# jasonleebrown/machisplin

Hardware: AMD Instinct MI355X
Metric: grid Mcells/s (ensemble+TPS predict) + TPS-solve GFLOP/s (higher is better)
Workload: dtype f64; 1 GPU; cfg3: 5000 stations, 3 covariates, 10000x10000 grid, 6-model ensemble + TPS residual correction; stations=5000, covariates=3 x float32 planes resident in HBM, rf_trees=500, tps_mode=global (one fit on all stations, GCV lambda, V73:748-753), parallelism=rowband1 + bcast(coef) + 1 all-gather

## Files before the change

### machisplin_amd/csrc/ensemble.hip

```cpp
#include <algorithm>
#include <atomic>
#include <cmath>
#include <cstdio>
#include <cstdlib>
#include <cstring>
#include <functional>
#include <mutex>
#include <type_traits>
#include <vector>
#include "common.h"
#include "devmath.h"

#include "ensemble_int.h"

namespace mhs {

__global__ __launch_bounds__(256) void lm_kernel(const double *__restrict__ coef, int p, StackDev s,
                                                 PredGeom g, double weight, int accumulate,
                                                 double *__restrict__ out) {
    const int64_t i = (int64_t)blockIdx.x * 256 + threadIdx.x;
    if (i >= (int64_t)g.nr * g.nc) return;
    const int row = (int)(i / g.nc), col = (int)(i - (int64_t)row * g.nc);
    double acc = coef[0];
    for (int j = 0; j < p; ++j) acc = acc + coef[j + 1] * predictor(s, g, j, row, col);
    emit(out, (int64_t)row * g.ld_out + col, acc, weight, accumulate);
}

__device__ __forceinline__ double nnet_sigmoid(double z) {
    if (z < -15.0) return 0.0;
    if (z > 15.0) return 1.0;
    return 1.0 / (1.0 + exp(-z));
}

template <int P>
__global__ __launch_bounds__(256) void nnet_kernel(const double *__restrict__ w, int H, double y_scale,
                                                   double y_shift, StackDev s, PredGeom g,
                                                   double weight, int accumulate,
                                                   double *__restrict__ out) {
    const int64_t i = (int64_t)blockIdx.x * 256 + threadIdx.x;
    if (i >= (int64_t)g.nr * g.nc) return;
    const int row = (int)(i / g.nc), col = (int)(i - (int64_t)row * g.nc);
    double x[P];
    bool na = false;
#pragma unroll
    for (int j = 0; j < P; ++j) { x[j] = predictor(s, g, j, row, col); na |= isnan(x[j]); }
    double acc = w[(P + 1) * H];
    for (int h = 0; h < H; ++h) {
        const double *wh = w + h * (P + 1);
        double z = wh[0];
#pragma unroll
        for (int j = 0; j < P; ++j) z = z + wh[1 + j] * x[j];
        acc = acc + w[(P + 1) * H + 1 + h] * nnet_sigmoid(z);
    }
    acc = acc * y_scale + y_shift;
    emit(out, (int64_t)row * g.ld_out + col, na ? NAN : acc, weight, accumulate);
}

__global__ __launch_bounds__(256) void earth_kernel(const double *__restrict__ coef,
                                                    const double *__restrict__ fcut,
                                                    const int *__restrict__ tstart,
                                                    const int *__restrict__ fvar,
                                                    const int *__restrict__ fdir, int nterms, int p,
                                                    StackDev s, PredGeom g, double weight, int accumulate,
                                                    double *__restrict__ out) {
    const int64_t i = (int64_t)blockIdx.x * 256 + threadIdx.x;
    if (i >= (int64_t)g.nr * g.nc) return;
    const int row = (int)(i / g.nc), col = (int)(i - (int64_t)row * g.nc);
    bool na = false;
    for (int j = 0; j < p; ++j) na |= isnan(predictor(s, g, j, row, col));
    double acc = 0.0;
    for (int k = 0; k < nterms; ++k) {
        double term = 1.0;
        for (int f = tstart[k]; f < tstart[k + 1]; ++f) {
            const double xv = predictor(s, g, fvar[f], row, col);
            const int d = fdir[f];
            const double fac = d == 2 ? xv : (d == 1 ? fmax(0.0, xv - fcut[f]) : fmax(0.0, fcut[f] - xv));
            term = term * fac;
        }
        acc = acc + coef[k] * term;
    }
    emit(out, (int64_t)row * g.ld_out + col, na ? NAN : acc, weight, accumulate);
}

struct SmallArgs {
    const double *lm_coef;
    const double *nn_w; int nn_H; double nn_scale, nn_shift;
    const double *ea_coef; const double *ea_cut; const int *ea_tstart, *ea_fvar, *ea_fdir; int ea_nterms;
    double w_lm, w_nn, w_ea;
};
template <int P>
__global__ __launch_bounds__(256) void small_members_kernel(SmallArgs a, StackDev s, PredGeom g, int accumulate,
                                                            double *__restrict__ out) {
    const int64_t i = (int64_t)blockIdx.x * 256 + threadIdx.x;
    if (i >= (int64_t)g.nr * g.nc) return;
    const int row = (int)(i / g.nc), col = (int)(i - (int64_t)row * g.nc);
    double x[P];
    bool na = false;
#pragma unroll
    for (int j = 0; j < P; ++j) { x[j] = predictor(s, g, j, row, col); na |= isnan(x[j]); }
    const int64_t o = (int64_t)row * g.ld_out + col;
    double v = accumulate ? out[o] : 0.0;
    bool first = !accumulate;
    auto add = [&](double pred, double w) { const double t = pred * w; v = first ? t : v + t; first = false; };
    if (a.lm_coef) {
        double acc = a.lm_coef[0];
#pragma unroll
        for (int j = 0; j < P; ++j) acc = acc + a.lm_coef[j + 1] * x[j];
        add(acc, a.w_lm);
    }
    if (a.nn_w) {
        double acc = a.nn_w[(P + 1) * a.nn_H];
        for (int h = 0; h < a.nn_H; ++h) {
            const double *wh = a.nn_w + h * (P + 1);
            double z = wh[0];
#pragma unroll
            for (int j = 0; j < P; ++j) z = z + wh[1 + j] * x[j];
            acc = acc + a.nn_w[(P + 1) * a.nn_H + 1 + h] * nnet_sigmoid(z);
        }
        acc = acc * a.nn_scale + a.nn_shift;
        add(na ? NAN : acc, a.w_nn);
    }
    if (a.ea_coef) {
        double acc = 0.0;
        for (int k = 0; k < a.ea_nterms; ++k) {
            double term = 1.0;
            for (int f = a.ea_tstart[k]; f < a.ea_tstart[k + 1]; ++f) {
                const double xv = predictor(s, g, a.ea_fvar[f], row, col);
                const int d = a.ea_fdir[f];
                const double fac = d == 2 ? xv : (d == 1 ? fmax(0.0, xv - a.ea_cut[f]) : fmax(0.0, a.ea_cut[f] - xv));
                term = term * fac;
            }
            acc = acc + a.ea_coef[k] * term;
        }
        add(na ? NAN : acc, a.w_ea);
    }
    out[o] = v;
}

constexpr int EXP_TAB_BITS = 12;
constexpr int EXP_TAB_N = 1 << EXP_TAB_BITS;
constexpr double EXP_SCALE = 4096.0 / 0.6931471805599453094;
__device__ __forceinline__ double table_exp_neg_acc(double u, const double *tab, double acc) {
    const double MAGIC = 0x1.8p52 + 1023.0 * EXP_TAB_N, NK = -EXP_RANGE * EXP_SCALE;
    const double t = fma(u, NK, MAGIC);
    const double kd = t - MAGIC;
    unsigned k8 = (unsigned)__double2loint(t) << 8;
    asm("" : "+v"(k8));
    const double r = fma(u, NK, -kd);
    const double mj = *(const double *)((const char *)tab + __builtin_amdgcn_ubfe(k8, 5, EXP_TAB_BITS + 3));
    const double sj = __hiloint2double((int)((k8 & 0xfff00000u) | (unsigned)__double2hiint(mj)), __double2loint(mj));
    const double C1 = 1.0 / EXP_SCALE, C2 = 0.5 / (EXP_SCALE * EXP_SCALE);
    double q = fma(r, C2, C1);
    q = fma(q, r, 1.0);
    return fma(sj, q, acc);
}

#if defined(__HIP_DEVICE_COMPILE__) && !defined(__GFX9__)
#error "table_exp_neg_acc_rt relies on v_lshlrev_b16 zeroing bits 16..31 of its destination (GFX9 encoding only)"
#endif
constexpr int EXP_TAB2_N = 2 * EXP_TAB_N;
__device__ __forceinline__ void rt_exp_table_stage(double *tab2, const double *__restrict__ gtab, int tid, int nthreads) {
    for (int i = tid; i < EXP_TAB2_N; i += nthreads) {
        const int j = i & (EXP_TAB_N - 1);
        const double e = gtab[j];
        tab2[i] = __hiloint2double((int)(((unsigned)__double2hiint(e) & 0x000fffffu) - ((unsigned)j << 8)), __double2loint(e));
    }
}
constexpr double RT_EXP_MAGIC = 0x1.8p52 + 1023.0 * EXP_TAB_N, RT_EXP_C1 = 1.0 / EXP_SCALE;
__device__ __forceinline__ void rt_exp_consts(double &magic, double &c1) {
    magic = RT_EXP_MAGIC; c1 = RT_EXP_C1;
    asm("" : "+v"(magic));
    asm("" : "+v"(c1));
}
__device__ __forceinline__ double table_exp_neg_acc_rt(double u, const double *tab2, double acc, double magic, double c1) {
    const double MAGIC = RT_EXP_MAGIC, NK = -EXP_RANGE * EXP_SCALE;
    const double t = fma(u, NK, magic);
    const double kd = t - MAGIC;
    const unsigned k = (unsigned)__double2loint(t);
    unsigned off;
    asm("v_lshlrev_b16 %0, 3, %1" : "=v"(off) : "v"(k));
    const double r = fma(u, NK, -kd);
    const double mj = *(const double *)((const char *)tab2 + off);
    const double sj = __hiloint2double((int)((k << 8) + (unsigned)__double2hiint(mj)), __double2loint(mj));
    const double C2 = 0.5 / (EXP_SCALE * EXP_SCALE);
    double q = fma(r, C2, c1);
    q = fma(q, r, 1.0);
    return fma(sj, q, acc);
}

template <int P, int R>
__global__ __launch_bounds__(256) void svr_kernel(const double *__restrict__ svp, int nsv, int stride,
                                                  int npos, const double *__restrict__ xcs,
                                                  const double *__restrict__ gtab, double sigma, double b,
                                                  double amax,
                                                  double y_center, double y_scale, StackDev s, PredGeom g,
                                                  double weight, int accumulate, double *__restrict__ out) {
    __shared__ double etab[EXP_TAB_N];
    for (int i = threadIdx.x; i < EXP_TAB_N; i += 256) {
        const double e = gtab[i];
        etab[i] = __hiloint2double(__double2hiint(e) & 0x000fffff, __double2loint(e));
    }
    __syncthreads();
    const int64_t total = (int64_t)g.nr * g.nc;
    const int64_t half = (total + R - 1) / R;
    const int64_t i0 = (int64_t)blockIdx.x * 256 + threadIdx.x;
    if (i0 >= half) return;
    double x[R][P], q[R], acc[R];
    bool na[R];
    int row[R], col[R];
#pragma unroll
    for (int c = 0; c < R; ++c) {
        int64_t i = i0 + c * half;
        if (i >= total) i = total - 1;
        row[c] = (int)(i / g.nc); col[c] = (int)(i - (int64_t)row[c] * g.nc);
        na[c] = false; q[c] = 0.0; acc[c] = 0.0;
#pragma unroll
        for (int j = 0; j < P; ++j) {
            const double xv = predictor(s, g, j, row[c], col[c]);
            na[c] |= isnan(xv);
            x[c][j] = (xv - xcs[j]) / xcs[P + j];
            q[c] = fma(x[c][j], x[c][j], q[c]);
        }
        q[c] = (sigma / EXP_RANGE) * q[c];
    }
    double accn[R];
#pragma unroll
    for (int c = 0; c < R; ++c) accn[c] = 0.0;
    auto sum_range = [&](int v0, int v1, double (&a)[R]) {
        for (int v = v0; v < v1; ++v) {
            const double *sp = svp + (int64_t)v * stride;
#pragma unroll
            for (int c = 0; c < R; ++c) {
                double arg = q[c] + fma(sp[P - 1], x[c][P - 1], sp[P]);
#pragma unroll
                for (int j = 0; j < P - 1; ++j) arg = fma(sp[j], x[c][j], arg);
                arg = fmin(fmax(arg, 0.0), 1.0);
                a[c] = table_exp_neg_acc(arg, etab, a[c]);
            }
        }
    };
    sum_range(0, npos, acc);
    sum_range(npos, nsv, accn);
#pragma unroll
    for (int c = 0; c < R; ++c) {
        const int64_t i = i0 + c * half;
        if (i < total) {
            const double pred = ((acc[c] - accn[c]) * amax - b) * y_scale + y_center;
            emit(out, (int64_t)row[c] * g.ld_out + col[c], na[c] ? NAN : pred, weight, accumulate);
        }
    }
}

__device__ __attribute__((noinline)) double svr_rt_exp_call(double z) { return exp(z); }
template <int P, int R, bool TAB2, bool EXPCALL>
__device__ __forceinline__ void svr_rt_tile(const double *__restrict__ svp, int nsv, int stride, int npos,
                                            const double *__restrict__ xcs, const double *etab, double *aw, double sigma, double b,
                                            double amax, double y_center, double y_scale, const StackDev &s, const PredGeom &g,
                                            int row, int tcol, int lane, double weight, int accumulate, double *__restrict__ out) {
    constexpr int CH = 128;
    double x[R][P], q[R], acc[R], accn[R];
    bool na[R], ok[R];
    int col[R];
#pragma unroll
    for (int c = 0; c < R; ++c) {
        const int cc = tcol + c * 64 + lane;
        ok[c] = cc < g.nc;
        col[c] = min(cc, g.nc - 1);
        na[c] = false; q[c] = 0.0; acc[c] = 0.0; accn[c] = 0.0;
#pragma unroll
        for (int j = 0; j < P; ++j) {
            const double xv = predictor(s, g, j, row, col[c]);
            na[c] |= isnan(xv);
            x[c][j] = (xv - xcs[j]) / xcs[P + j];
            q[c] = fma(x[c][j], x[c][j], q[c]);
        }
        q[c] = (sigma / EXP_RANGE) * q[c];
    }
    const double xlat = x[0][P - 1];
    double qhi = -1.0, qlo = 2e300;
#pragma unroll
    for (int c = 0; c < R; ++c) { qhi = fmax(qhi, q[c]); qlo = fmin(qlo, q[c]); }
#pragma unroll
    for (int o = 32; o > 0; o >>= 1) { qhi = fmax(qhi, __shfl_xor(qhi, o)); qlo = fmin(qlo, __shfl_xor(qlo, o)); }
    const bool fold = __builtin_amdgcn_readfirstlane((int)(qhi - qlo <= 0.5)) != 0;
    const double S = fold ? qhi : 0.0;
    double magic = 0.0, c1 = 0.0;
    if constexpr (TAB2) rt_exp_consts(magic, c1);
    auto sum_range = [&](int v0, int v1, double (&a)[R], auto folded) {
        constexpr bool FOLD = decltype(folded)::value;
        auto pair = [&](const double *sp, const double ap) {
#pragma unroll
            for (int c = 0; c < R; ++c) {
                double arg = FOLD ? ap : q[c] + ap;
#pragma unroll
                for (int j = 0; j < P - 1; ++j) arg = fma(sp[j], x[c][j], arg);
                arg = fmin(fmax(arg, 0.0), 1.0);
                a[c] = TAB2 ? table_exp_neg_acc_rt(arg, etab, a[c], magic, c1) : table_exp_neg_acc(arg, etab, a[c]);
            }
        };
        for (int vb = v0; vb < v1; vb += CH) {
            const int n = min(CH, v1 - vb);
            __builtin_amdgcn_wave_barrier();
            for (int e = lane; e < n; e += 64) {
                const double *sp = svp + (int64_t)(vb + e) * stride;
                aw[e] = fma(sp[P - 1], xlat, sp[P]) + S;
            }
            __builtin_amdgcn_wave_barrier();
            const double *sp = svp + (int64_t)vb * stride;
            const double *ar = aw;
            int e = 0;
            for (; e + 4 <= n; e += 4) {
#pragma unroll
                for (int k = 0; k < 4; ++k) pair(sp + (int64_t)k * stride, ar[e + k]);
                sp += (int64_t)4 * stride;
            }
            for (; e < n; ++e) { pair(sp, ar[e]); sp += stride; }
        }
    };
    if (fold) {
        sum_range(0, npos, acc, std::true_type());
        sum_range(npos, nsv, accn, std::true_type());
    } else {
        sum_range(0, npos, acc, std::false_type());
        sum_range(npos, nsv, accn, std::false_type());
    }
#pragma unroll
    for (int c = 0; c < R; ++c)
        if (ok[c]) {
            const double back = fold ? (EXPCALL ? svr_rt_exp_call(EXP_RANGE * (S - q[c])) : exp(EXP_RANGE * (S - q[c]))) : 1.0;
            const double pred = ((acc[c] - accn[c]) * back * amax - b) * y_scale + y_center;
            emit(out, (int64_t)row * g.ld_out + col[c], na[c] ? NAN : pred, weight, accumulate);
        }
}

template <int P, int R, bool TAB2>
__device__ __forceinline__ void svr_rt_run(int64_t tile, const double *__restrict__ svp, int nsv, int stride, int npos,
                                           const double *__restrict__ xcs, const double *etab, double *aw, double sigma, double b,
                                           double amax, double y_center, double y_scale, const StackDev &s, const PredGeom &g,
                                           int tiles_per_row, int lane, double weight, int accumulate, double *__restrict__ out) {
    const int row = (int)(tile / tiles_per_row), tcol = (int)(tile - (int64_t)row * tiles_per_row) * (64 * R);
    svr_rt_tile<P, R, TAB2, true>(svp, nsv, stride, npos, xcs, etab, aw, sigma, b, amax, y_center, y_scale, s, g, row, tcol, lane, weight,
                                  accumulate, out);
}
template <int NW, bool TAB2>
__device__ __forceinline__ void svr_rt_stage(double *etab, const double *__restrict__ gtab) {
    if constexpr (TAB2) rt_exp_table_stage(etab, gtab, threadIdx.x, 64 * NW);
    else
        for (int i = threadIdx.x; i < EXP_TAB_N; i += 64 * NW) {
            const double e = gtab[i];
            etab[i] = __hiloint2double(__double2hiint(e) & 0x000fffff, __double2loint(e));
        }
}

template <int P, int R, int NW, bool TAB2>
__global__ __launch_bounds__(64 * NW) void svr_rt_kernel(const double *__restrict__ svp, int nsv, int stride,
                                                         int npos, const double *__restrict__ xcs,
                                                         const double *__restrict__ gtab, double sigma, double b,
                                                         double amax, double y_center, double y_scale, StackDev s, PredGeom g,
                                                         int tiles_per_row, double weight, int accumulate, double *__restrict__ out) {
    __shared__ double etab[TAB2 ? EXP_TAB2_N : EXP_TAB_N];
    __shared__ double aw[NW][128];
    svr_rt_stage<NW, TAB2>(etab, gtab);
    __syncthreads();
    const int wave = threadIdx.x >> 6, lane = threadIdx.x & 63;
    const int64_t ntiles = (int64_t)g.nr * tiles_per_row;
    const int64_t tile = (int64_t)blockIdx.x * NW + wave;
    if (tile >= ntiles) return;
    const int row = (int)(tile / tiles_per_row), tcol = (int)(tile - (int64_t)row * tiles_per_row) * (64 * R);
    svr_rt_tile<P, R, TAB2, false>(svp, nsv, stride, npos, xcs, etab, aw[wave], sigma, b, amax, y_center, y_scale, s, g, row, tcol, lane,
                                   weight, accumulate, out);
}

struct SvrRtScalars {
    int nsv, stride, npos, tiles_per_row; double sigma, b, amax, y_center, y_scale;
    StackDev s; PredGeom g; double weight; int accumulate;
};
constexpr int SVR_RT_SCALARS_AT = 5 * sizeof(void *);
static_assert(alignof(SvrRtScalars) <= 8, "svr_rt_resident_kernel: `sc` does not follow the pointers without padding");
static_assert(sizeof(PredGeom) == 64 && sizeof(StackDev) == 48 && sizeof(SvrRtScalars) == 184,
              "svr_rt_resident_kernel copies PredGeom / StackDev field by field: update the copies and these sizes together");
inline void svr_rt_field_counts(const PredGeom &g, const StackDev &s) {
    const auto &[g0, g1, g2, g3, g4, g5, g6, g7, g8] = g;
    const auto &[s0, s1, s2, s3, s4, s5, s6, s7] = s;
    (void)g0; (void)g1; (void)g2; (void)g3; (void)g4; (void)g5; (void)g6; (void)g7; (void)g8;
    (void)s0; (void)s1; (void)s2; (void)s3; (void)s4; (void)s5; (void)s6; (void)s7;
}
template <int P, int R, int NW, bool TAB2, int WPS>
__global__ __launch_bounds__(64 * NW, WPS) void svr_rt_resident_kernel(const double *__restrict__ svp, const double *__restrict__ xcs,
                                                                  const double *__restrict__ gtab, double *__restrict__ out,
                                                                  unsigned long long *__restrict__ pool, SvrRtScalars sc) {
    __shared__ double etab[TAB2 ? EXP_TAB2_N : EXP_TAB_N];
    __shared__ double aw[NW][128];
    svr_rt_stage<NW, TAB2>(etab, gtab);
    __syncthreads();
    const int wave = threadIdx.x >> 6, lane = threadIdx.x & 63;
    typedef const __attribute__((address_space(4))) char *KBytes;
    typedef const __attribute__((address_space(4))) SvrRtScalars *KScalars;
    for (;;) {
        KScalars k = (KScalars)((KBytes)__builtin_amdgcn_kernarg_segment_ptr() + SVR_RT_SCALARS_AT);
        asm volatile("" : "+s"(k));
        unsigned long long t = 0;
        if (lane == 0) t = atomicAdd(pool, 1ull);
        const int64_t tile = (int64_t)(((unsigned long long)(unsigned)__builtin_amdgcn_readfirstlane((int)(t >> 32)) << 32) |
                                       (unsigned)__builtin_amdgcn_readfirstlane((int)t));
        const PredGeom g = {k->g.xmin, k->g.ymax, k->g.xres, k->g.yres, k->g.r0, k->g.c0, k->g.nr, k->g.nc, k->g.ld_out};
        if (tile >= (int64_t)g.nr * k->tiles_per_row) return;
        const StackDev s = {k->s.data, k->s.C, k->s.dtype, k->s.plane_stride, k->s.ld, k->s.nodata, k->s.has_nodata, k->s.all_from_planes};
        svr_rt_run<P, R, TAB2>(tile, svp, k->nsv, k->stride, k->npos, xcs, etab, aw[wave], k->sigma, k->b, k->amax,
                               k->y_center, k->y_scale, s, g, k->tiles_per_row, lane, k->weight, k->accumulate, out);
    }
}

template <bool GBM, bool LDS_NODES, int R, bool NA_ONLY, bool SPLIT = false>
__global__ __launch_bounds__(256) void tree_kernel(const Node *__restrict__ gnodes,
                                                   const int *__restrict__ tree_off,
                                                   const TreeChunk *__restrict__ chunks, int n_chunks,
                                                   int n_trees, double init_f, int p, StackDev s,
                                                   PredGeom g, double weight, int accumulate,
                                                   double *__restrict__ out, const unsigned *__restrict__ na_gate = nullptr) {
    extern __shared__ __attribute__((aligned(16))) char smem[];
    if (NA_ONLY && na_gate && na_gate[1] == 0u) return;
    double *xs = (double *)smem;
    Node *lnodes = (Node *)(smem + (size_t)p * R * 256 * sizeof(double));
    const int64_t total = (int64_t)g.nr * g.nc;
    const int64_t half = (total + R - 1) / R;
    const int64_t i0 = (int64_t)blockIdx.x * 256 + threadIdx.x;
    int row[R], col[R];
    bool na[R];
    double acc[R];
#pragma unroll
    for (int c = 0; c < R; ++c) {
        int64_t i = i0 + c * half;
        if (i >= total) i = total - 1;
        if (i < 0) i = 0;
        row[c] = (int)(i / g.nc); col[c] = (int)(i - (int64_t)row[c] * g.nc);
        na[c] = false; acc[c] = 0.0;
        for (int j = 0; j < p; ++j) {
            const double xv = predictor(s, g, j, row[c], col[c]);
            na[c] |= isnan(xv);
            xs[(j * R + c) * 256 + threadIdx.x] = xv;
        }
    }
    if (NA_ONLY) {
        bool any = false;
#pragma unroll
        for (int c = 0; c < R; ++c) any |= na[c] && i0 < half && (i0 + c * half) < total;
        if (!__syncthreads_or(any)) return;
    }
    int ch_begin = 0, ch_end = n_chunks;
    if (SPLIT) {
        const int per = (n_chunks + (int)gridDim.y - 1) / (int)gridDim.y;
        ch_begin = min((int)blockIdx.y * per, n_chunks);
        ch_end = min(ch_begin + per, n_chunks);
    }
    for (int ch = ch_begin; ch < ch_end; ++ch) {
        const TreeChunk tc = chunks[ch];
        if (LDS_NODES) {
            __syncthreads();
            const int4 *src = (const int4 *)(gnodes + tc.node_begin);
            int4 *dst = (int4 *)lnodes;
            for (int e = threadIdx.x; e < tc.node_count; e += 256) dst[e] = src[e];
            __syncthreads();
        }
        for (int t = tc.first_tree; t < tc.first_tree + tc.n_trees; ++t) {
            const int tbase = LDS_NODES ? tree_off[t] - tc.node_begin : tree_off[t];
#pragma unroll
            for (int c = 0; c < R; ++c) {
                if (NA_ONLY && !na[c]) continue;
                Node nd;
                if constexpr (LDS_NODES) nd = lnodes[tbase]; else nd = gnodes[tbase];
                while (nd.var >= 0) {
                    const double xv = xs[(nd.var * R + c) * 256 + threadIdx.x];
                    unsigned nxt;
                    if (GBM) nxt = isnan(xv) ? nd.missing : (xv < nd.val ? nd.left : nd.right);
                    else nxt = (xv <= nd.val) ? nd.left : nd.right;
                    if constexpr (LDS_NODES) nd = lnodes[tbase + nxt]; else nd = gnodes[tbase + nxt];
                }
                acc[c] = acc[c] + nd.val;
            }
        }
    }
    if (SPLIT) {
#pragma unroll
        for (int c = 0; c < R; ++c) {
            const int64_t i = i0 + c * half;
            if (i0 < half && i < total) out[(int64_t)blockIdx.y * total + i] = (!GBM && na[c]) ? NAN : acc[c];
        }
        return;
    }
#pragma unroll
    for (int c = 0; c < R; ++c) {
        const int64_t i = i0 + c * half;
        if (i0 < half && i < total && (!NA_ONLY || na[c])) {
            double pred;
            if (GBM) pred = init_f + acc[c];
            else pred = na[c] ? NAN : acc[c] / (double)n_trees;
            emit(out, (int64_t)row[c] * g.ld_out + col[c], pred, weight, accumulate);
        }
    }
}


__global__ __launch_bounds__(256) void na_collect_kernel(StackDev s, PredGeom g, unsigned cap, unsigned *__restrict__ list) {
    const int64_t total = (int64_t)g.nr * g.nc;
    const int64_t i = (int64_t)blockIdx.x * 256 + threadIdx.x;
    if (i >= total) return;
    const int row = (int)(i / g.nc), col = (int)(i - (int64_t)row * g.nc);
    bool na = false;
    for (int j = 0; j < s.C; ++j) na |= isnan(predictor(s, g, j, row, col));
    if (na) {
        const unsigned slot = atomicAdd(&list[0], 1u);
        if (slot < cap) list[2 + slot] = (unsigned)i;
        else list[1] = 1u;
    }
}
template <bool LDS_NODES>
__global__ __launch_bounds__(256) void gbm_na_list_kernel(const Node *__restrict__ gnodes, const int *__restrict__ tree_off,
                                                          const TreeChunk *__restrict__ chunks, int n_chunks, double init_f, int p,
                                                          StackDev s, PredGeom g, double weight, int accumulate,
                                                          double *__restrict__ out, const unsigned *__restrict__ list, unsigned cap) {
    extern __shared__ __attribute__((aligned(16))) char smem[];
    if (list[1]) return;
    double *xs = (double *)smem;
    Node *lnodes = (Node *)(smem + (size_t)p * 256 * sizeof(double));
    const unsigned count = min(list[0], cap);
    for (unsigned base = blockIdx.x * 256u; base < count; base += gridDim.x * 256u) {
        const bool live = base + threadIdx.x < count;
        const int64_t i = list[2 + (live ? base + threadIdx.x : base)];
        const int row = (int)(i / g.nc), col = (int)(i - (int64_t)row * g.nc);
        for (int j = 0; j < p; ++j) xs[j * 256 + threadIdx.x] = predictor(s, g, j, row, col);
        double acc = 0.0;
        for (int ch = 0; ch < n_chunks; ++ch) {
            const TreeChunk tc = chunks[ch];
            if (LDS_NODES) {
                __syncthreads();
                const int4 *src = (const int4 *)(gnodes + tc.node_begin);
                int4 *dst = (int4 *)lnodes;
                for (int e = threadIdx.x; e < tc.node_count; e += 256) dst[e] = src[e];
                __syncthreads();
            }
            for (int t = tc.first_tree; t < tc.first_tree + tc.n_trees; ++t) {
                const int tbase = LDS_NODES ? tree_off[t] - tc.node_begin : tree_off[t];
                Node nd;
                if constexpr (LDS_NODES) nd = lnodes[tbase]; else nd = gnodes[tbase];
                while (nd.var >= 0) {
                    const double xv = xs[nd.var * 256 + threadIdx.x];
                    const unsigned nxt = isnan(xv) ? nd.missing : (xv < nd.val ? nd.left : nd.right);
                    if constexpr (LDS_NODES) nd = lnodes[tbase + nxt]; else nd = gnodes[tbase + nxt];
                }
                acc = acc + nd.val;
            }
        }
        if (live) emit(out, (int64_t)row * g.ld_out + col, init_f + acc, weight, accumulate);
        __syncthreads();
    }
}


template <bool HI>
__device__ __forceinline__ void pred_bits(float2v &b01, float2v &b23, const float2v k01, const float2v k23,
                                          const unsigned long long cpair) {
    if (!HI)
        asm("v_pk_add_f32 %0, %2, %4 op_sel_hi:[1,0] clamp\n\t"
            "v_pk_add_f32 %1, %3, %4 op_sel_hi:[1,0] clamp"
            : "=&v"(b01), "=&v"(b23) : "v"(k01), "v"(k23), "s"(cpair));
    else
        asm("v_pk_add_f32 %0, %2, %4 op_sel:[0,1] op_sel_hi:[1,1] clamp\n\t"
            "v_pk_add_f32 %1, %3, %4 op_sel:[0,1] op_sel_hi:[1,1] clamp"
            : "=&v"(b01), "=&v"(b23) : "v"(k01), "v"(k23), "s"(cpair));
}


template <int S>
__global__ __launch_bounds__(256) void gbm_lut_kernel(const double *__restrict__ lut,
                                                      const int *__restrict__ meta,
                                                      const void *__restrict__ sorted, int key64,
                                                      const int *__restrict__ sorted_off, int n_trees_padded,
                                                      double init_f, int p, StackDev s, PredGeom g,
                                                      double weight, int accumulate,
                                                      double *__restrict__ out) {
    static_assert((LUT_CHUNK << S) * sizeof(double) >= LUT_COARSE * sizeof(float), "coarse table must fit");
    extern __shared__ __attribute__((aligned(16))) char smem[];
    float *keys = (float *)smem;
    double *slut = (double *)(smem + (size_t)p * 256 * LUT_R * sizeof(float));
    float *coarse = (float *)slut;
    const int64_t total = (int64_t)g.nr * g.nc;
    const int64_t quarter = (total + LUT_R - 1) / LUT_R;
    const int64_t i0 = (int64_t)blockIdx.x * 256 + threadIdx.x;
    int row[LUT_R], col[LUT_R];
    bool na[LUT_R];
    double acc[LUT_R];
#pragma unroll
    for (int c = 0; c < LUT_R; ++c) {
        int64_t i = i0 + c * quarter;
        if (i >= total) i = total - 1;
        row[c] = (int)(i / g.nc); col[c] = (int)(i - (int64_t)row[c] * g.nc);
        na[c] = false; acc[c] = 0.0;
    }
    for (int j = 0; j < p; ++j) {
        float r[LUT_R];
        lut_ranks<LUT_R, 256>(j, sorted, key64, sorted_off, coarse, s, g, row, col, na, r);
#pragma unroll
        for (int c = 0; c < LUT_R; ++c) keys[(j * 256 + threadIdx.x) * LUT_R + c] = -r[c];
    }
    const char *kbase = (const char *)(keys + threadIdx.x * LUT_R);
    constexpr unsigned A0_BITS = (unsigned)(127 + 23 - S) << 23;
    unsigned lut_base = (unsigned)p * 256u * LUT_R * (unsigned)sizeof(float) - 0x58000000u;
    asm volatile("" : "+s"(lut_base));
    for (int t0 = 0; t0 < n_trees_padded; t0 += LUT_CHUNK) {
        __syncthreads();
        for (int e = threadIdx.x; e < (LUT_CHUNK << S); e += 256) slut[e] = lut[((int64_t)t0 << S) + e];
        __syncthreads();
#pragma unroll 2
        for (int t = 0; t < LUT_CHUNK; ++t) {
            const int *m = meta + (int64_t)(t0 + t) * LUT_META_DW;
            const unsigned long long *mc = (const unsigned long long *)m;
            const unsigned long long a0 = A0_BITS + ((unsigned)t << S);
            float2v a01, a23, b01, b23;
            {
                const float4 k = *(const float4 *)(kbase + m[6]);
                pred_bits<false>(b01, b23, float2v{k.x, k.y}, float2v{k.z, k.w}, mc[0]);
                asm("v_pk_fma_f32 %0, %2, 2.0, %3 op_sel_hi:[0,0,1]\n\t"
                    "v_pk_fma_f32 %1, %2, 2.0, %4 op_sel_hi:[0,0,1]"
                    : "=&v"(a01), "=&v"(a23) : "s"(a0), "v"(b01), "v"(b23));
            }
#pragma unroll
            for (int q = 1; q < S; ++q) {
                const float4 k = *(const float4 *)(kbase + m[6 + q]);
                if (q & 1) pred_bits<true>(b01, b23, float2v{k.x, k.y}, float2v{k.z, k.w}, mc[q >> 1]);
                else pred_bits<false>(b01, b23, float2v{k.x, k.y}, float2v{k.z, k.w}, mc[q >> 1]);
                asm("v_pk_fma_f32 %0, %0, 2.0, %2 op_sel_hi:[1,0,1]\n\t"
                    "v_pk_fma_f32 %1, %1, 2.0, %3 op_sel_hi:[1,0,1]"
                    : "+v"(a01), "+v"(a23) : "v"(b01), "v"(b23));
            }
            acc[0] = acc[0] + *(const double *)(smem + (__float_as_uint(a01.x) * 8u + lut_base));
            acc[1] = acc[1] + *(const double *)(smem + (__float_as_uint(a01.y) * 8u + lut_base));
            acc[2] = acc[2] + *(const double *)(smem + (__float_as_uint(a23.x) * 8u + lut_base));
            acc[3] = acc[3] + *(const double *)(smem + (__float_as_uint(a23.y) * 8u + lut_base));
        }
    }
#pragma unroll
    for (int c = 0; c < LUT_R; ++c) {
        const int64_t i = i0 + c * quarter;
        if (i0 < quarter && i < total && !na[c])
            emit(out, (int64_t)row[c] * g.ld_out + col[c], init_f + acc[c], weight, accumulate);
    }
}

typedef float float32v __attribute__((ext_vector_type(32)));
constexpr int LUT_REG_P = 8;

#define MHS_LUT_LEVEL(IDX, CP, SEL)                                                   \
    "s_set_gpr_idx_idx %[" IDX "]\n\t"                                               \
    "v_pk_add_f32 %[b01], v[64:65], %[" CP "] " SEL " clamp\n\t"                     \
    "v_pk_add_f32 %[b23], v[66:67], %[" CP "] " SEL " clamp\n\t"                     \
    "v_pk_fma_f32 %[a01], 2.0, %[a01], %[b01] op_sel_hi:[0,1,1]\n\t"                 \
    "v_pk_fma_f32 %[a23], 2.0, %[a23], %[b23] op_sel_hi:[0,1,1]\n\t"
#define MHS_SEL_LO "op_sel_hi:[1,0]"
#define MHS_SEL_HI "op_sel:[0,1] op_sel_hi:[1,1]"

template <int S>
__device__ __forceinline__ void lut_tree_reg(float2v &a01, float2v &a23, const float32v &keys, const int *m,
                                             const unsigned long long a0) {
    const unsigned long long *mc = (const unsigned long long *)m;
    const unsigned long long c01 = mc[0], c23 = mc[1], c45 = mc[2];
    const int i0 = m[6] >> 10, i1 = m[7] >> 10, i2 = m[8] >> 10, i3 = m[9] >> 10, i4 = m[10] >> 10;
    float2v b01, b23;
    if (S == 5) {
        asm("s_set_gpr_idx_on %[i0], 0x1\n\t"
            "v_pk_add_f32 %[b01], v[64:65], %[c01] op_sel_hi:[1,0] clamp\n\t"
            "v_pk_add_f32 %[b23], v[66:67], %[c01] op_sel_hi:[1,0] clamp\n\t"
            "v_pk_fma_f32 %[a01], 2.0, %[a0], %[b01] op_sel_hi:[0,0,1]\n\t"
            "v_pk_fma_f32 %[a23], 2.0, %[a0], %[b23] op_sel_hi:[0,0,1]\n\t"
            MHS_LUT_LEVEL("i1", "c01", MHS_SEL_HI)
            MHS_LUT_LEVEL("i2", "c23", MHS_SEL_LO)
            MHS_LUT_LEVEL("i3", "c23", MHS_SEL_HI)
            MHS_LUT_LEVEL("i4", "c45", MHS_SEL_LO)
            "s_set_gpr_idx_off"
            : [a01] "=&v"(a01), [a23] "=&v"(a23), [b01] "=&v"(b01), [b23] "=&v"(b23)
            : "{v[64:95]}"(keys), [i0] "s"(i0), [i1] "s"(i1), [i2] "s"(i2), [i3] "s"(i3), [i4] "s"(i4),
              [c01] "s"(c01), [c23] "s"(c23), [c45] "s"(c45), [a0] "s"(a0));
    } else {
        const int i5 = m[11] >> 10;
        asm("s_set_gpr_idx_on %[i0], 0x1\n\t"
            "v_pk_add_f32 %[b01], v[64:65], %[c01] op_sel_hi:[1,0] clamp\n\t"
            "v_pk_add_f32 %[b23], v[66:67], %[c01] op_sel_hi:[1,0] clamp\n\t"
            "v_pk_fma_f32 %[a01], 2.0, %[a0], %[b01] op_sel_hi:[0,0,1]\n\t"
            "v_pk_fma_f32 %[a23], 2.0, %[a0], %[b23] op_sel_hi:[0,0,1]\n\t"
            MHS_LUT_LEVEL("i1", "c01", MHS_SEL_HI)
            MHS_LUT_LEVEL("i2", "c23", MHS_SEL_LO)
            MHS_LUT_LEVEL("i3", "c23", MHS_SEL_HI)
            MHS_LUT_LEVEL("i4", "c45", MHS_SEL_LO)
            MHS_LUT_LEVEL("i5", "c45", MHS_SEL_HI)
            "s_set_gpr_idx_off"
            : [a01] "=&v"(a01), [a23] "=&v"(a23), [b01] "=&v"(b01), [b23] "=&v"(b23)
            : "{v[64:95]}"(keys), [i0] "s"(i0), [i1] "s"(i1), [i2] "s"(i2), [i3] "s"(i3), [i4] "s"(i4), [i5] "s"(i5),
              [c01] "s"(c01), [c23] "s"(c23), [c45] "s"(c45), [a0] "s"(a0));
    }
}

template <int S, bool K64>
__global__ __launch_bounds__(256, 5) void gbm_lutreg_kernel(const double *__restrict__ lut,
                                                         const int *__restrict__ meta,
                                                         const void *__restrict__ sorted, int key64,
                                                         const int *__restrict__ sorted_off, int n_trees_padded,
                                                         double init_f, int p, StackDev s, PredGeom g,
                                                         double weight, int accumulate,
                                                         double *__restrict__ out) {
    static_assert((LUT_CHUNK << S) * sizeof(double) >= LUT_COARSE * sizeof(float), "coarse table must fit");
    extern __shared__ __attribute__((aligned(16))) char smem[];
    double *slut = (double *)smem;
    float *coarse = (float *)smem;
    const int64_t total = (int64_t)g.nr * g.nc;
    const int64_t quarter = (total + LUT_R - 1) / LUT_R;
    const int64_t i0 = (int64_t)blockIdx.x * 256 + threadIdx.x;
    int row[LUT_R], col[LUT_R];
    bool na[LUT_R];
    double acc[LUT_R];
#pragma unroll
    for (int c = 0; c < LUT_R; ++c) {
        int64_t i = i0 + c * quarter;
        if (i >= total) i = total - 1;
        row[c] = (int)(i / g.nc); col[c] = (int)(i - (int64_t)row[c] * g.nc);
        na[c] = false; acc[c] = 0.0;
    }
    float32v keys;
#pragma unroll
    for (int j = 0; j < LUT_REG_P; ++j) {
        float r[LUT_R] = {0.f, 0.f, 0.f, 0.f};
        if (j < p) {
            if constexpr (K64) lut_ranks_t<LUT_R, 256, double>(j, (const double *)sorted, sorted_off, (double *)coarse, s, g, row, col, na, r);
            else lut_ranks_t<LUT_R, 256, float>(j, (const float *)sorted, sorted_off, coarse, s, g, row, col, na, r);
        }
#pragma unroll
        for (int c = 0; c < LUT_R; ++c) keys[j * LUT_R + c] = -r[c];
    }
    constexpr unsigned A0_BITS = (unsigned)(127 + 23 - S) << 23;
    unsigned lut_base = 0u - 0x58000000u;
    asm volatile("" : "+s"(lut_base));
    for (int t0 = 0; t0 < n_trees_padded; t0 += LUT_CHUNK) {
        __syncthreads();
        for (int e = threadIdx.x; e < (LUT_CHUNK << S); e += 256) slut[e] = lut[((int64_t)t0 << S) + e];
        __syncthreads();
#pragma unroll 2
        for (int t = 0; t < LUT_CHUNK; ++t) {
            float2v a01, a23;
            lut_tree_reg<S>(a01, a23, keys, meta + (int64_t)(t0 + t) * LUT_META_DW, A0_BITS + ((unsigned)t << S));
            acc[0] = acc[0] + *(const double *)(smem + (__float_as_uint(a01.x) * 8u + lut_base));
            acc[1] = acc[1] + *(const double *)(smem + (__float_as_uint(a01.y) * 8u + lut_base));
            acc[2] = acc[2] + *(const double *)(smem + (__float_as_uint(a23.x) * 8u + lut_base));
            acc[3] = acc[3] + *(const double *)(smem + (__float_as_uint(a23.y) * 8u + lut_base));
        }
    }
#pragma unroll
    for (int c = 0; c < LUT_R; ++c) {
        const int64_t i = i0 + c * quarter;
        if (i0 < quarter && i < total && !na[c])
            emit(out, (int64_t)row[c] * g.ld_out + col[c], init_f + acc[c], weight, accumulate);
    }
}

constexpr int LUT_RT_DW = 16;
constexpr int LUT_RT_MAXK = 2;
typedef unsigned long long u64x8 __attribute__((ext_vector_type(8)));

constexpr int GBC_PROBE_BLOCKS = 4, GBC_PROBE_CHUNKS = 4, GBC_PROBE_SLOTS = 1024;
__device__ __forceinline__ bool gbc_coherent_pays(const int *__restrict__ probe) {
    long long cost = 0, cnt = 0;
#pragma unroll
    for (int b = 0; b < GBC_PROBE_BLOCKS; ++b) { cost += probe[2 * b]; cnt += probe[2 * b + 1]; }
    return cost < 83 * cnt;
}
template <bool K64>
__global__ __launch_bounds__(256, 5) void gbm_lutreg_rt_kernel(const double *__restrict__ lut,
                                                            const u64x8 *__restrict__ meta,
                                                            const void *__restrict__ sorted,
                                                            const int *__restrict__ sorted_off, int n_trees_padded,
                                                            double init_f, int p, StackDev s, PredGeom g, int tiles_per_row,
                                                            double weight, int accumulate,
                                                            double *__restrict__ out, const int *__restrict__ probe) {
    constexpr int S = 5;
    static_assert((LUT_CHUNK << S) * sizeof(double) >= LUT_COARSE * sizeof(float), "coarse table must fit");
    extern __shared__ __attribute__((aligned(16))) char smem[];
    if (probe && gbc_coherent_pays(probe)) return;
    double *slut = (double *)smem;
    float *coarse = (float *)smem;
    const int lane = threadIdx.x & 63;
    const int64_t ntiles = (int64_t)g.nr * tiles_per_row;
    int64_t tile = (int64_t)blockIdx.x * 4 + (threadIdx.x >> 6);
    const bool live = tile < ntiles;
    if (!live) tile = ntiles - 1;
    const int trow = (int)(tile / tiles_per_row), tcol = (int)(tile - (int64_t)trow * tiles_per_row) * (64 * LUT_R);
    int row[LUT_R], col[LUT_R];
    bool na[LUT_R], ok[LUT_R];
    double acc[LUT_R];
#pragma unroll
    for (int c = 0; c < LUT_R; ++c) {
        const int cc = tcol + c * 64 + lane;
        ok[c] = live && cc < g.nc;
        row[c] = trow; col[c] = min(cc, g.nc - 1);
        na[c] = false; acc[c] = 0.0;
    }
    float32v keys;
    int latv = 0;
#pragma unroll
    for (int j = 0; j < LUT_REG_P; ++j) {
        float r[LUT_R] = {0.f, 0.f, 0.f, 0.f};
        if (j < p) {
            if constexpr (K64) lut_ranks_t<LUT_R, 256, double>(j, (const double *)sorted, sorted_off, (double *)coarse, s, g, row, col, na, r);
            else lut_ranks_t<LUT_R, 256, float>(j, (const float *)sorted, sorted_off, coarse, s, g, row, col, na, r);
            if (j == s.C + 1) latv = (int)r[0];
        }
#pragma unroll
        for (int c = 0; c < LUT_R; ++c) keys[j * LUT_R + c] = -r[c];
    }
    const int latrank = __builtin_amdgcn_readfirstlane(latv);
    unsigned lut_base = 0u - 0x58000000u;
    asm volatile("" : "+s"(lut_base));
    for (int t0 = 0; t0 < n_trees_padded; t0 += LUT_CHUNK) {
        __syncthreads();
        for (int e = threadIdx.x; e < (LUT_CHUNK << S); e += 256) slut[e] = lut[((int64_t)t0 << S) + e];
        __syncthreads();
        const u64x8 *mp = meta + t0;
        asm volatile(
#include "gbm_rt_loop.inc"
            : [acc0] "+v"(acc[0]), [acc1] "+v"(acc[1]), [acc2] "+v"(acc[2]), [acc3] "+v"(acc[3])
            : "{v[64:95]}"(keys), [mp] "s"(mp), [lat] "s"(latrank), [lb] "s"(lut_base)
            : "memory", "scc",
              "s36", "s37", "s38", "s39", "s40", "s41", "s42", "s43", "s44", "s45", "s46", "s47", "s48", "s49", "s50", "s51",
              "s52", "s53", "s54", "s55", "s56", "s57", "s58", "s59", "s60", "s61", "s62", "s63", "s64", "s65", "s66", "s67",
              "s68", "s69", "s70", "s71", "s72", "s73", "s74",
              "v40", "v41", "v42", "v43", "v44", "v45", "v46", "v47", "v48", "v49", "v50", "v51", "v52", "v53", "v54", "v55",
              "v56", "v57", "v58", "v59");
    }
#pragma unroll
    for (int c = 0; c < LUT_R; ++c)
        if (ok[c] && !na[c]) emit(out, (int64_t)row[c] * g.ld_out + col[c], init_f + acc[c], weight, accumulate);
}


constexpr int GBC_WAVES = 16;
__device__ __forceinline__ double gbc_lds_f64(unsigned a) { return *(__attribute__((address_space(3))) const double *)(uintptr_t)a; }
typedef float float4v __attribute__((ext_vector_type(4)));
template <bool K64, bool PROBE = false>
__global__ __launch_bounds__(1024) void gbm_coherent_kernel(const double *__restrict__ lut, const unsigned *__restrict__ cls,
                                                            const void *__restrict__ sorted, const int *__restrict__ sorted_off,
                                                            int n_trees_padded, double init_f, int p, StackDev s, PredGeom g,
                                                            int tiles_per_row, double weight, int accumulate,
                                                            double *__restrict__ out, int *__restrict__ probe, int tile16,
                                                            const int *__restrict__ axis_rank, int axis_ncol) {
    constexpr int S = 5, CH = LUT_CHUNK, CLS_STRIDE = 384, R = LUT_R;
    if (!PROBE && probe && !gbc_coherent_pays(probe)) return;
    if (PROBE) n_trees_padded = min(n_trees_padded, GBC_PROBE_CHUNKS * CH);
    static_assert(R == 4, "four cells per lane: two packed predicate instructions");
    static_assert((CH << S) * sizeof(double) >= LUT_COARSE * sizeof(float), "coarse table must fit");
    extern __shared__ __attribute__((aligned(16))) char smem[];
    double *slut = (double *)smem;
    unsigned *scls = (unsigned *)(smem + 2 * (CH << S) * sizeof(double));
    int2 *srange = (int2 *)(scls + 2 * CLS_STRIDE);
    float *coarse = (float *)smem;
    if ((unsigned)(uintptr_t)(__attribute__((address_space(3))) char *)smem != 0u) __builtin_trap();
    const int tid = threadIdx.x, wave = tid >> 6, lane = tid & 63;
    const int TW = tile16 ? 16 : 64, TH = tile16 ? 4 * R : R;
    const int roff = (int)(g.r0 % TH), coff = (int)(g.c0 % TW);
    const int64_t ntiles = (int64_t)((g.nr + roff + TH - 1) / TH) * tiles_per_row;
    int64_t tile = (int64_t)blockIdx.x * GBC_WAVES + wave;
    if (PROBE) tile = ntiles >= GBC_PROBE_BLOCKS * GBC_WAVES ? tile * (ntiles / (GBC_PROBE_BLOCKS * GBC_WAVES)) : tile % ntiles;
    const bool live = tile < ntiles;
    if (!live) tile = ntiles - 1;
    const int trow = (int)(tile / tiles_per_row) * TH - roff + (tile16 ? (lane >> 4) * R : 0);
    const int tcol = (int)(tile % tiles_per_row) * TW - coff + (tile16 ? (lane & 15) : lane);
    int row[R], col[R];
    bool na[R], ok[R];
    double acc[R];
#pragma unroll
    for (int c = 0; c < R; ++c) {
        const int rr = trow + c, cc = tcol;
        ok[c] = live && cc >= 0 && cc < g.nc && rr >= 0 && rr < g.nr;
        row[c] = min(max(rr, 0), g.nr - 1); col[c] = min(max(cc, 0), g.nc - 1);
        na[c] = false; acc[c] = 0.0;
    }
    float32v keys;
#pragma unroll
    for (int j = 0; j < LUT_REG_P; ++j) {
        float r[R] = {0.f, 0.f, 0.f, 0.f};
        if (j < p) {
            if (axis_rank && j >= s.C && !s.all_from_planes) {
#pragma unroll
                for (int c = 0; c < R; ++c)
                    r[c] = (float)(j == s.C ? axis_rank[g.c0 + col[c]] : axis_rank[(int64_t)axis_ncol + g.r0 + row[c]]);
            } else if constexpr (K64) lut_ranks_t<R, 1024, double>(j, (const double *)sorted, sorted_off, (double *)coarse, s, g, row, col, na, r);
            else lut_ranks_t<R, 1024, float>(j, (const float *)sorted, sorted_off, coarse, s, g, row, col, na, r);
        }
#pragma unroll
        for (int c = 0; c < R; ++c) keys[j * R + c] = -r[c];
        int mn = 0x7fffffff, mx = -1;
#pragma unroll
        for (int c = 0; c < R; ++c)
            if (!na[c]) { mn = min(mn, (int)r[c]); mx = max(mx, (int)r[c]); }
#pragma unroll
        for (int o = 32; o > 0; o >>= 1) { mn = min(mn, __shfl_xor(mn, o)); mx = max(mx, __shfl_xor(mx, o)); }
        if (lane == 0) srange[wave * 8 + j] = make_int2(mn, mx);
    }
    __syncthreads();
    for (int e = tid; e < (CH << S); e += 1024) slut[e] = lut[e];
    if (tid < CH * S) scls[tid] = cls[tid];
    __syncthreads();
    double usum = 0.0;
    int pcost = 0;
    for (int t0 = 0, buf = 0; t0 < n_trees_padded; t0 += CH, buf ^= 1) {
        const bool more = t0 + CH < n_trees_padded;
        double pre0 = 0.0, pre1 = 0.0;
        unsigned prec = 0u;
        if (more) {
            const double *ln = lut + ((int64_t)(t0 + CH) << S);
            pre0 = ln[tid]; pre1 = ln[tid + 1024];
            if (tid < CH * S) prec = cls[(int64_t)(t0 + CH) * S + tid];
        }
        const unsigned *cw = scls + buf * CLS_STRIDE + lane * S;
        const double *L = slut + buf * (CH << S) + (lane << S);
        unsigned w[S];
        int2 mm[S];
#pragma unroll
        for (int q = 0; q < S; ++q) w[q] = cw[q];
#pragma unroll
        for (int q = 0; q < S; ++q) mm[q] = srange[wave * 8 + (int)(w[q] & 7u)];
        unsigned known = 0u, smask = 0u;
#pragma unroll
        for (int q = 0; q < S; ++q) {
            const int c = (int)(w[q] >> 3);
            const bool all1 = mm[q].y < c, all0 = mm[q].x >= c;
            if (all1) known |= 16u >> q;
            if (!(all1 || all0)) smask |= 16u >> q;
        }
        const unsigned nstr = (unsigned)__popc(smask);
        if (PROBE) {
            if (nstr) pcost += 85 + 26 * (int)nstr;
            if (more) {
                double *ld = slut + (buf ^ 1) * (CH << S);
                ld[tid] = pre0; ld[tid + 1024] = pre1;
                if (tid < CH * S) scls[(buf ^ 1) * CLS_STRIDE + tid] = prec;
            }
            __syncthreads();
            continue;
        }
        const double B = L[known];
        const bool single = nstr == 1u, pair = nstr == 2u, multi = nstr >= 3u;
        if (!multi) usum = usum + B;
        double d1 = 0.0, d2 = 0.0, d12 = 0.0;
        unsigned f1 = 0u, f2 = 0u;
        if (single || pair) {
            const int pos1 = 31 - __clz((int)(smask | 1u));
            const unsigned p1 = 1u << pos1;
            f1 = cw[S - 1 - pos1];
            const double A1 = L[known + p1];
            d1 = (A1 - B) * 128.0;
            if (pair) {
                const int pos2 = 31 - __clz((int)((smask & ~p1) | 1u));
                const unsigned p2 = 1u << pos2;
                f2 = cw[S - 1 - pos2];
                const double A2 = L[known + p2], A12 = L[known + p1 + p2];
                d2 = (A2 - B) * 128.0;
                d12 = (((A12 - A1) - A2) + B) * 16384.0;
            }
            f1 = __float_as_uint((float)(int)(f1 >> 3)) | (f1 & 7u);
            f2 = __float_as_uint((float)(int)(f2 >> 3)) | (f2 & 7u);
        }
#define MHS_GBC_RL(x) __builtin_amdgcn_readlane((int)(x), t)
#define MHS_GBC_RLD(x) __hiloint2double(__builtin_amdgcn_readlane(__double2hiint(x), t), __builtin_amdgcn_readlane(__double2loint(x), t))
#define MHS_GBC_THR(fw) (int)((unsigned)(fw) & ~7u)
#define MHS_GBC_VO(fw) (int)(((unsigned)(fw) & 7u) << 2)
#define MHS_GBC_BITS(h0, h1, h2, h3, vo, cc)                                                                 \
        asm volatile("s_set_gpr_idx_on %[v], 0x1\n\t"                                                        \
                     "v_add_f32_e64 %[a], v64, %[c] clamp\n\t"                                               \
                     "v_add_f32_e64 %[b], v65, %[c] clamp\n\t"                                               \
                     "v_add_f32_e64 %[d], v66, %[c] clamp\n\t"                                               \
                     "v_add_f32_e64 %[e], v67, %[c] clamp\n\t"                                               \
                     "s_set_gpr_idx_off"                                                                     \
                     : [a] "=&v"(h0), [b] "=&v"(h1), [d] "=&v"(h2), [e] "=&v"(h3)                            \
                     : "{v[64:95]}"(keys), [v] "s"(vo), [c] "s"(cc));
        for (unsigned long long m1 = __builtin_amdgcn_ballot_w64(single); m1; m1 &= m1 - 1ull) {
            const int t = (int)__builtin_ctzll(m1);
            const int fw = MHS_GBC_RL(f1);
            const int cc = MHS_GBC_THR(fw), vo = MHS_GBC_VO(fw);
            const double e1 = MHS_GBC_RLD(d1);
            int h[R];
            MHS_GBC_BITS(h[0], h[1], h[2], h[3], vo, cc)
#pragma unroll
            for (int c = 0; c < R; ++c) acc[c] = fma(__hiloint2double(h[c], 0), e1, acc[c]);
        }
        for (unsigned long long mp = __builtin_amdgcn_ballot_w64(pair); mp; mp &= mp - 1ull) {
            const int t = (int)__builtin_ctzll(mp);
            const int fa = MHS_GBC_RL(f1), fb = MHS_GBC_RL(f2);
            const int c1 = MHS_GBC_THR(fa), v1 = MHS_GBC_VO(fa), c2 = MHS_GBC_THR(fb), v2 = MHS_GBC_VO(fb);
            const double e1 = MHS_GBC_RLD(d1), e2 = MHS_GBC_RLD(d2), e12 = MHS_GBC_RLD(d12);
            int h[R], k[R];
            MHS_GBC_BITS(h[0], h[1], h[2], h[3], v1, c1)
            MHS_GBC_BITS(k[0], k[1], k[2], k[3], v2, c2)
#pragma unroll
            for (int c = 0; c < R; ++c) {
                const double b1 = __hiloint2double(h[c], 0), b2 = __hiloint2double(k[c], 0);
                acc[c] = fma(b1, e1, acc[c]);
                acc[c] = fma(b2, fma(b1, e12, e2), acc[c]);
            }
        }
#undef MHS_GBC_BITS
#undef MHS_GBC_RLD
        const unsigned abase = (unsigned)buf * (unsigned)((CH << S) * sizeof(double)) - 0x58000000u;
        unsigned long long m2 = __builtin_amdgcn_ballot_w64(multi);
        unsigned wf[S];
#pragma unroll
        for (int q = 0; q < S; ++q) wf[q] = w[q];
        if (m2) {
#pragma unroll
            for (int q = 0; q < S; ++q) wf[q] = __float_as_uint((float)(int)(w[q] >> 3)) | (w[q] & 7u);
        }
        for (; m2; m2 &= m2 - 1ull) {
            const int t = (int)__builtin_ctzll(m2);
            const unsigned sm = (unsigned)MHS_GBC_RL(smask);
            const float a0 = __uint_as_float(0x4B000000u + ((unsigned)t << S) + (unsigned)MHS_GBC_RL(known));
            float2v s01 = {a0, a0}, s23 = {a0, a0};
#pragma unroll
            for (int q = 0; q < S; ++q) {
                if (sm & (16u >> q)) {
                    const int fw = MHS_GBC_RL(wf[q]);
                    const unsigned long long cc = (unsigned)MHS_GBC_THR(fw);
                    const int vo = MHS_GBC_VO(fw);
                    const unsigned long long wb = (127u + (unsigned)(S - 1 - q)) << 23;
                    float2v b01, b23;
                    asm volatile("s_set_gpr_idx_on %[vo], 0x1\n\t"
                                 "v_pk_add_f32 %[b01], v[64:65], %[cc] op_sel_hi:[1,0] clamp\n\t"
                                 "v_pk_add_f32 %[b23], v[66:67], %[cc] op_sel_hi:[1,0] clamp\n\t"
                                 "s_set_gpr_idx_off\n\t"
                                 "v_pk_fma_f32 %[s01], %[b01], %[wb], %[s01] op_sel_hi:[1,0,1]\n\t"
                                 "v_pk_fma_f32 %[s23], %[b23], %[wb], %[s23] op_sel_hi:[1,0,1]"
                                 : [s01] "+v"(s01), [s23] "+v"(s23), [b01] "=&v"(b01), [b23] "=&v"(b23)
                                 : "{v[64:95]}"(keys), [vo] "s"(vo), [cc] "s"(cc), [wb] "s"(wb));
                }
            }
            acc[0] = acc[0] + gbc_lds_f64(__float_as_uint(s01.x) * 8u + abase);
            acc[1] = acc[1] + gbc_lds_f64(__float_as_uint(s01.y) * 8u + abase);
            acc[2] = acc[2] + gbc_lds_f64(__float_as_uint(s23.x) * 8u + abase);
            acc[3] = acc[3] + gbc_lds_f64(__float_as_uint(s23.y) * 8u + abase);
        }
#undef MHS_GBC_VO
#undef MHS_GBC_THR
#undef MHS_GBC_RL
        if (more) {
            double *ld = slut + (buf ^ 1) * (CH << S);
            ld[tid] = pre0; ld[tid + 1024] = pre1;
            if (tid < CH * S) scls[(buf ^ 1) * CLS_STRIDE + tid] = prec;
        }
        __syncthreads();
    }
    if (PROBE) {
        int *tot = (int *)srange;
        __syncthreads();
        if (tid == 0) tot[0] = 0;
        __syncthreads();
#pragma unroll
        for (int o = 32; o > 0; o >>= 1) pcost += __shfl_xor(pcost, o);
        if (lane == 0) atomicAdd(tot, pcost);
        __syncthreads();
        if (tid == 0) { probe[2 * blockIdx.x] = tot[0]; probe[2 * blockIdx.x + 1] = GBC_WAVES * n_trees_padded; }
        return;
    }
#pragma unroll
    for (int o = 32; o > 0; o >>= 1) usum = usum + __shfl_xor(usum, o);
#pragma unroll
    for (int c = 0; c < R; ++c)
        if (ok[c] && !na[c]) emit(out, (int64_t)row[c] * g.ld_out + col[c], init_f + (acc[c] + usum), weight, accumulate);
}
static size_t gbc_lds_bytes() {
    return 2 * ((size_t)LUT_CHUNK << 5) * sizeof(double) + 2 * 384 * sizeof(unsigned) + GBC_WAVES * 8 * sizeof(int2);
}

__global__ __launch_bounds__(256) void gbm_staged_points_kernel(const Node *__restrict__ nodes, const int *__restrict__ tree_off,
                                                                int n_trees, double init_f, const double *__restrict__ X,
                                                                int64_t n, int step, double *__restrict__ out) {
    const int64_t i = (int64_t)blockIdx.x * 256 + threadIdx.x;
    if (i >= n) return;
    double acc = 0.0;
    for (int t = 0; t < n_trees; ++t) {
        const int tb = tree_off[t];
        Node nd = nodes[tb];
        while (nd.var >= 0) {
            const double xv = X[(int64_t)nd.var * n + i];
            const unsigned nxt = isnan(xv) ? nd.missing : (xv < nd.val ? nd.left : nd.right);
            nd = nodes[tb + nxt];
        }
        acc = acc + nd.val;
        if ((t + 1) % step == 0) out[(int64_t)((t + 1) / step - 1) * n + i] = init_f + acc;
    }
}

struct ResidualArgs { double w[8]; };
__global__ __launch_bounds__(256) void residual_points_kernel(const double *__restrict__ pred, const double *__restrict__ resp,
                                                              int64_t n, int n_models, ResidualArgs a, double wt_total,
                                                              double *__restrict__ out) {
    const int64_t i = (int64_t)blockIdx.x * 256 + threadIdx.x;
    if (i >= n) return;
    const double y = resp[i];
    double res = (y - pred[i]) * a.w[0];
    for (int k = 1; k < n_models; ++k) res = res + (y - pred[(int64_t)k * n + i]) * a.w[k];
    out[i] = res / wt_total;
}

__global__ __launch_bounds__(256) void scale_add_kernel(const double *__restrict__ a, double divisor,
                                                        const double *__restrict__ b,
                                                        double *__restrict__ out, int64_t n) {
    const int64_t i = (int64_t)blockIdx.x * 256 + threadIdx.x;
    if (i >= n) return;
    double v = a[i] / divisor;
    if (b) v = v + b[i];
    out[i] = v;
}

__global__ __launch_bounds__(256) void scale_window_kernel(double *__restrict__ out, int nr, int nc,
                                                           int64_t ld, double divisor) {
    const int64_t i = (int64_t)blockIdx.x * 256 + threadIdx.x;
    if (i >= (int64_t)nr * nc) return;
    const int row = (int)(i / nc), col = (int)(i - (int64_t)row * nc);
    out[(int64_t)row * ld + col] = out[(int64_t)row * ld + col] / divisor;
}


template <int P>
static void launch_nnet(const mhs_model *m, const StackDev &s, const PredGeom &g, double w, int acc,
                        double *out, hipStream_t st, unsigned blocks) {
    hipLaunchKernelGGL((nnet_kernel<P>), dim3(blocks), dim3(256), 0, st, m->dpar, m->n0, m->s0, m->s1, s, g, w, acc, out);
}
constexpr bool svr_rt_tab2(int P) { return P <= 5; }
constexpr int svr_rt_waves_per_simd(int P) { return P <= 5 ? 4 : 3; }
constexpr int svr_rt_waves(int P) { return svr_rt_tab2(P) ? 16 : 4; }

static std::mutex svr_pool_mu[MAX_SLOTS];
static int svr_pool_take(Context &c, hipStream_t st, int *idx, unsigned long long **counter) {
    if (!c.svr_pool) {
        for (hipEvent_t &e : c.svr_pool_ev)
            if (!e) MHS_HIP(hipEventCreateWithFlags(&e, hipEventDisableTiming));
        MHS_HIP(hipMalloc((void **)&c.svr_pool, sizeof(unsigned long long) * SVR_POOL_SLOTS));
    }
    *idx = (int)(c.svr_pool_next++ % SVR_POOL_SLOTS);
    *counter = c.svr_pool + *idx;
    MHS_HIP(hipStreamWaitEvent(st, c.svr_pool_ev[*idx], 0));
    MHS_HIP(hipMemsetAsync(*counter, 0, sizeof(unsigned long long), st));
    return MHS_OK;
}

template <int P>
static int launch_svr(const mhs_model *m, const StackDev &s, const PredGeom &g, double w, int acc,
                      double *out, hipStream_t st, int64_t total) {
    constexpr int R = 3;
    const int tpr = (g.nc + 64 * R - 1) / (64 * R);
    if (!s.all_from_planes && P == s.C + 2 && P >= 3 && !getenv("MHS_SVR_NO_ROWTILE") && (double)g.nc >= 0.93 * (double)tpr * (64 * R)) {
        const int64_t ntiles = (int64_t)g.nr * tpr;
        constexpr int NW = svr_rt_waves(P);
        const int64_t covering = (ntiles + NW - 1) / NW;
        if constexpr (svr_rt_tab2(P)) {
            auto kern = svr_rt_resident_kernel<P, R, NW, true, svr_rt_waves_per_simd(P)>;
            Context &c = ctx();
            std::lock_guard<std::mutex> lk(svr_pool_mu[current_slot()]);
            int &per_cu = c.svr_rt_blocks_per_cu[P];
            if (per_cu == 0) {
                int n = 0;
                MHS_HIP(hipOccupancyMaxActiveBlocksPerMultiprocessor(&n, (const void *)kern, 64 * NW, 0));
                per_cu = std::max(1, n);
            }
            const int64_t resident = (int64_t)(c.n_cu > 0 ? c.n_cu : 256) * per_cu;
            int idx = 0;
            unsigned long long *counter = nullptr;
            if (int rc = svr_pool_take(c, st, &idx, &counter)) return rc;
            const SvrRtScalars sc = {m->n0, m->n1, m->n2, tpr, m->s1, m->s0, m->s4, m->s2, m->s3, s, g, w, acc};
            hipLaunchKernelGGL(kern, dim3((unsigned)std::min(resident, covering)), dim3(64 * NW), 0, st,
                               m->dpar, m->dpar + (size_t)m->n0 * m->n1, c.exp_tab, out, counter, sc);
            MHS_HIP(hipEventRecord(c.svr_pool_ev[idx], st));
            return MHS_OK;
        }
        else {
            hipLaunchKernelGGL((svr_rt_kernel<P, R, NW, false>), dim3((unsigned)covering), dim3(64 * NW), 0, st,
                               m->dpar, m->n0, m->n1, m->n2, m->dpar + (size_t)m->n0 * m->n1, ctx().exp_tab, m->s1, m->s0, m->s4,
                               m->s2, m->s3, s, g, tpr, w, acc, out);
            return MHS_OK;
        }
    }
    const int64_t half = (total + R - 1) / R;
    hipLaunchKernelGGL((svr_kernel<P, R>), dim3((unsigned)((half + 255) / 256)), dim3(256), 0, st,
                       m->dpar, m->n0, m->n1, m->n2, m->dpar + (size_t)m->n0 * m->n1, ctx().exp_tab, m->s1, m->s0, m->s4,
                       m->s2, m->s3,
                       s, g, w, acc, out);
    return MHS_OK;
}

#define MHS_DISPATCH_P(P_, CALL)                                                     \
    switch (P_) {                                                                    \
        case 2: CALL(2); break; case 3: CALL(3); break; case 4: CALL(4); break;      \
        case 5: CALL(5); break; case 6: CALL(6); break; case 7: CALL(7); break;      \
        case 8: CALL(8); break; case 9: CALL(9); break; case 10: CALL(10); break;    \
        case 11: CALL(11); break; case 12: CALL(12); break;                          \
        default: set_error("predict: p = %d exceeds the %d predictors this build supports for nnet/ksvm", P_, PMAX); \
                 return MHS_ERR_INVALID;                                             \
    }

template <bool GBM>
__global__ __launch_bounds__(256) void tree_finalize_kernel(const double *__restrict__ part, int shares, int64_t total,
                                                            double init_f, int n_trees, PredGeom g, double weight,
                                                            int accumulate, double *__restrict__ out) {
    const int64_t i = (int64_t)blockIdx.x * 256 + threadIdx.x;
    if (i >= total) return;
    double acc = 0.0;
    for (int y = 0; y < shares; ++y) acc = acc + part[(int64_t)y * total + i];
    const int row = (int)(i / g.nc), col = (int)(i - (int64_t)row * g.nc);
    emit(out, (int64_t)row * g.ld_out + col, GBM ? init_f + acc : acc / (double)n_trees, weight, accumulate);
}

constexpr int64_t TREE_SPLIT_MAX_CELLS = 16384;
constexpr int TREE_SPLIT_SHARES = 64;

template <typename K, typename... Args>
static int launch_tree_kernel(const mhs_model *m, K lds_kern, K global_kern, dim3 blocks, size_t xs_bytes, hipStream_t st, Args... args) {
    const K kern = m->lds_ok ? lds_kern : global_kern;
    const size_t bytes = xs_bytes + (m->lds_ok ? (size_t)m->max_chunk_nodes * sizeof(Node) : 0);
    MHS_HIP(hipFuncSetAttribute((const void *)kern, hipFuncAttributeMaxDynamicSharedMemorySize, (int)bytes));
    hipLaunchKernelGGL(kern, blocks, dim3(256), bytes, st, args...);
    return MHS_OK;
}

template <bool GBM, bool NA_ONLY>
static int launch_trees(const mhs_model *m, const StackDev &s, const PredGeom &g, double w, int acc,
                        double *out, hipStream_t st, int64_t total, const unsigned *na_gate = nullptr) {
    const size_t xs_bytes = (size_t)m->p * TREE_R * 256 * sizeof(double);
    if (xs_bytes > LDS_MAX) {
        const size_t xs1 = (size_t)m->p * 256 * sizeof(double);
        const auto kern = tree_kernel<GBM, false, 1, NA_ONLY>;
        MHS_HIP(hipFuncSetAttribute((const void *)kern, hipFuncAttributeMaxDynamicSharedMemorySize, (int)xs1));
        hipLaunchKernelGGL(kern, dim3((unsigned)((total + 255) / 256)), dim3(256), xs1, st, m->nodes, m->tree_off, m->chunks, m->n_chunks,
                           m->n_trees, m->init_f, m->p, s, g, w, acc, out, na_gate);
        return MHS_OK;
    }
    const int64_t half = (total + TREE_R - 1) / TREE_R;
    const unsigned blocks = (unsigned)((half + 255) / 256);
    if (!NA_ONLY && m->lds_ok && total <= TREE_SPLIT_MAX_CELLS && m->n_chunks >= 4) {
        const int shares = std::min(m->n_chunks, TREE_SPLIT_SHARES);
        mhs_model *mm = const_cast<mhs_model *>(m);
        if (!mm->split_scratch) MHS_HIP(hipMalloc((void **)&mm->split_scratch, sizeof(double) * TREE_SPLIT_MAX_CELLS * TREE_SPLIT_SHARES));
        auto kern = tree_kernel<GBM, true, TREE_R, false, true>;
        if (int rc = launch_tree_kernel(m, kern, kern, dim3(blocks, (unsigned)shares), xs_bytes, st, m->nodes, m->tree_off, m->chunks,
                                        m->n_chunks, m->n_trees, m->init_f, m->p, s, g, w, acc, mm->split_scratch, (const unsigned *)nullptr))
            return rc;
        hipLaunchKernelGGL(tree_finalize_kernel<GBM>, dim3((unsigned)((total + 255) / 256)), dim3(256), 0, st,
                           mm->split_scratch, shares, total, m->init_f, m->n_trees, g, w, acc, out);
        return MHS_OK;
    }
    return launch_tree_kernel(m, tree_kernel<GBM, true, TREE_R, NA_ONLY>, tree_kernel<GBM, false, TREE_R, NA_ONLY>, dim3(blocks), xs_bytes, st,
                              m->nodes, m->tree_off, m->chunks, m->n_chunks, m->n_trees, m->init_f, m->p, s, g, w, acc, out, na_gate);
}

template <typename KT>
static int build_lut_meta_t(mhs_model *m, const mhs_grid &grid, int C) {
    const int S = m->lut_S;
    std::vector<KT> tkey((size_t)m->n_trees * S, (KT)0);
    std::vector<std::vector<KT>> sorted((size_t)m->p);
    for (int t = 0; t < m->n_trees; ++t) {
        for (int q = 0; q < S; ++q) {
            const int v = m->lut_var[(size_t)t * S + q];
            if (v < 0) continue;
            const KT tk = split_tkey<KT, false>(v, C, m->lut_thr[(size_t)t * S + q], grid);
            tkey[(size_t)t * S + q] = tk;
            sorted[(size_t)v].push_back(tk);
        }
    }
    std::vector<int> off;
    std::vector<KT> flat;
    sort_unique(sorted, off, flat);
    for (int v = 0; v < m->p; ++v)
        if (sorted[(size_t)v].size() >= ((size_t)1 << 24)) { set_error("gbm: too many distinct split values"); return MHS_ERR_INVALID; }
    if (int rc = publish_axis_ranks(m, sorted, C, grid)) return rc;
    std::vector<int> meta((size_t)m->n_trees_padded * LUT_META_DW, 0);
    const float never = -33554432.f;
    for (int t = 0; t < m->n_trees_padded; ++t) {
        int *mt = &meta[(size_t)t * LUT_META_DW];
        for (int q = 0; q < 6; ++q) { memcpy(&mt[q], &never, 4); mt[6 + q] = 0; }
        if (t >= m->n_trees) continue;
        for (int q = 0; q < S; ++q) {
            const int v = m->lut_var[(size_t)t * S + q];
            if (v < 0) continue;
            const std::vector<KT> &sv = sorted[(size_t)v];
            const KT tk = tkey[(size_t)t * S + q];
            const float c = (float)((std::lower_bound(sv.begin(), sv.end(), tk) - sv.begin()) + 1);
            memcpy(&mt[q], &c, 4);
            mt[6 + q] = v * 256 * LUT_R * (int)sizeof(float);
        }
    }
    if (m->p <= LUT_REG_P && S == 5 && !m->lut_host.empty()) {
        const int lat = C + 1 < m->p ? C + 1 : -2;
        std::vector<int> rmeta(((size_t)m->n_trees_padded + 1) * LUT_RT_DW, 0);
        std::vector<double> rlut(m->lut_host.size(), 0.0);
        for (int t = 0; t <= m->n_trees_padded; ++t) {
            int *mt = &rmeta[(size_t)t * LUT_RT_DW];
            for (int q = 0; q < 5; ++q) { memcpy(&mt[q], &never, 4); mt[6 + q] = 0; mt[11 + q] = 0; }
            mt[5] = S - LUT_RT_MAXK;
            if (t >= m->n_trees) continue;
            int perm[6], K = 0, n = 0;
            bool first[6] = {false, false, false, false, false, false};
            for (int q = 0; q < S && K < LUT_RT_MAXK; ++q) {
                const int v = m->lut_var[(size_t)t * S + q];
                if (v < 0 || v == lat) { perm[n++] = q; first[q] = true; ++K; }
            }
            for (int q = 0; q < S; ++q) if (!first[q]) perm[n++] = q;
            for (int i = 0; i < S; ++i) {
                const int q = perm[i], v = m->lut_var[(size_t)t * S + q];
                if (v < 0) continue;
                const std::vector<KT> &sv = sorted[(size_t)v];
                const int c = (int)(std::lower_bound(sv.begin(), sv.end(), tkey[(size_t)t * S + q]) - sv.begin()) + 1;
                if (i < K) mt[11 + i] = c;
                else { const float cf = (float)c; memcpy(&mt[i - K], &cf, 4); mt[6 + i - K] = v * LUT_R; }
            }
            mt[5] = S - K;
            for (int b = 0; b < (1 << S); ++b) {
                int bo = 0;
                for (int i = 0; i < S; ++i) bo |= ((b >> (S - 1 - i)) & 1) << (S - 1 - perm[i]);
                rlut[((size_t)t << S) + b] = m->lut_host[((size_t)t << S) + bo];
            }
        }
        if (int rc = publish(m, rlut, &m->lut_rt)) return rc;
        if (int rc = publish(m, rmeta, &m->lut_rt_meta)) return rc;
        std::vector<unsigned> cw((size_t)m->n_trees_padded * 5, 0u);
        for (int t = 0; t < m->n_trees; ++t)
            for (int q = 0; q < S; ++q) {
                const int v = m->lut_var[(size_t)t * S + q];
                if (v < 0) continue;
                const std::vector<KT> &sv = sorted[(size_t)v];
                const unsigned c = (unsigned)(std::lower_bound(sv.begin(), sv.end(), tkey[(size_t)t * S + q]) - sv.begin()) + 1u;
                cw[(size_t)t * 5 + q] = (c << 3) | (unsigned)v;
            }
        bool fits = true;
        for (int v = 0; v < m->p; ++v) fits = fits && sorted[(size_t)v].size() < ((size_t)1 << 20);
        if (fits) { if (int rc = publish(m, cw, &m->lut_cls)) return rc; }
        else if (m->lut_cls) { m->retired.push_back((void *)m->lut_cls); m->lut_cls = nullptr; }
    }
    if (int rc = publish(m, flat, (KT **)&m->lut_sorted)) return rc;
    if (int rc = publish(m, off, &m->lut_sorted_off)) return rc;
    return publish(m, meta, &m->lut_meta);
}

static int build_lut_meta(mhs_model *m, const mhs_grid &grid, int C, int key64, TreeTables *tt) {
    std::lock_guard<std::mutex> lk(m->mu);
    if (!(m->lut_meta && same_meta(m, grid, C, key64))) {
        if (int rc = key64 ? build_lut_meta_t<double>(m, grid, C) : build_lut_meta_t<float>(m, grid, C)) return rc;
        m->meta_grid = grid; m->meta_C = C; m->meta_key64 = key64;
    }
    *tt = TreeTables{m->lut_sorted, m->lut_sorted_off, m->lut_meta, nullptr, nullptr, m->lut_rt, m->lut_rt_meta, m->lut_cls, m->axis_rank, m->axis_ncol};
    return MHS_OK;
}

static int launch_gbm_na(const mhs_model *m, const StackDev &s, const PredGeom &g, double w, int acc, double *out, hipStream_t st,
                         int64_t total) {
    if (total >= (1LL << 32)) return launch_trees<true, true>(m, s, g, w, acc, out, st, total);
    mhs_model *mm = const_cast<mhs_model *>(m);
    const unsigned slot = mm->na_next.fetch_add(1) % 4;
    const size_t want = (size_t)std::max<int64_t>(4096, total / 8);
    unsigned *list = nullptr;
    unsigned cap = 0;
    {
        std::lock_guard<std::mutex> lk(mm->mu);
        if (!mm->na_done[slot]) MHS_HIP(hipEventCreateWithFlags(&mm->na_done[slot], hipEventDisableTiming));
        else if (mm->na_stream[slot] != st) MHS_HIP(hipStreamWaitEvent(st, mm->na_done[slot], 0));
        if (mm->na_cap[slot] < want) {
            if (mm->na_list[slot]) {
                MHS_HIP(hipEventSynchronize(mm->na_done[slot]));
                MHS_HIP(hipStreamSynchronize(st));
                (void)hipFree(mm->na_list[slot]); mm->na_list[slot] = nullptr; mm->na_cap[slot] = 0;
            }
            MHS_HIP(hipMalloc((void **)&mm->na_list[slot], sizeof(unsigned) * (want + 2)));
            mm->na_cap[slot] = want;
        }
        list = mm->na_list[slot];
        cap = (unsigned)mm->na_cap[slot];
        mm->na_stream[slot] = st;
    }
    MHS_HIP(hipMemsetAsync(list, 0, 2 * sizeof(unsigned), st));
    hipLaunchKernelGGL(na_collect_kernel, dim3((unsigned)((total + 255) / 256)), dim3(256), 0, st, s, g, cap, list);
    const unsigned lblocks = (unsigned)std::min<int64_t>(2048, (total / 8 + 255) / 256 + 1);
    if (int rc = launch_tree_kernel(m, gbm_na_list_kernel<true>, gbm_na_list_kernel<false>, dim3(lblocks), (size_t)m->p * 256 * sizeof(double), st,
                                    m->nodes, m->tree_off, m->chunks, m->n_chunks, m->init_f, m->p, s, g, w, acc, out, list, cap))
        return rc;
    if (int rc = launch_trees<true, true>(m, s, g, w, acc, out, st, total, list)) return rc;
    MHS_HIP(hipGetLastError());
    {
        std::lock_guard<std::mutex> lk(mm->mu);
        MHS_HIP(hipEventRecord(mm->na_done[slot], st));
    }
    return MHS_OK;
}

static bool gbm_lut_applies(const mhs_model *m, const StackDev &s, const mhs_grid *grid) {
    return grid && m->lut_S > 0 && !s.all_from_planes && !getenv("MHS_TREES_GENERIC") &&
           (size_t)m->p * 256 * LUT_R * 4 + ((size_t)LUT_CHUNK << m->lut_S) * 8 <= LDS_LIMIT;
}

static int launch_gbm_lut(const mhs_model *m, const StackDev &s, const PredGeom &g, const mhs_grid &grid,
                          double w, int acc, double *out, hipStream_t st, int64_t total) {
    const int key64 = s.dtype == MHS_F64;
    TreeTables tt;
    if (int rc = build_lut_meta(const_cast<mhs_model *>(m), grid, s.C, key64, &tt)) return rc;
    const int64_t quarter = (total + LUT_R - 1) / LUT_R;
    const unsigned blocks = (unsigned)((quarter + 255) / 256);
    const size_t lut_bytes = ((size_t)LUT_CHUNK << m->lut_S) * sizeof(double);
    const bool in_regs = m->p <= LUT_REG_P;
    const int tpr = (g.nc + 64 * LUT_R - 1) / (64 * LUT_R);
    const int ctw = 16, cth = 4 * LUT_R;
    const int ctpr = (int)((g.nc + g.c0 % ctw + ctw - 1) / ctw);
    const bool rt_ok = in_regs && m->lut_S == 5 && tt.lut_rt && (double)g.nc >= 0.93 * (double)tpr * (64 * LUT_R);
    const bool coh_ok = in_regs && m->lut_S == 5 && tt.lut_cls && g.nr >= 2 * LUT_R && (double)g.nc >= 0.8 * (double)ctpr * ctw &&
                        !getenv("MHS_GBM_NO_COHERENT");
    int *probe = nullptr;
    if (coh_ok && rt_ok && total >= (1 << 20) && !getenv("MHS_GBM_FORCE_COHERENT")) {
        mhs_model *mm = const_cast<mhs_model *>(m);
        {
            std::lock_guard<std::mutex> lk(mm->mu);
            if (!mm->gbm_probe) MHS_HIP(hipMalloc(&mm->gbm_probe, sizeof(int) * 2 * GBC_PROBE_BLOCKS * GBC_PROBE_SLOTS));
        }
        probe = mm->gbm_probe + (size_t)(mm->gbm_probe_next.fetch_add(1) % GBC_PROBE_SLOTS) * 2 * GBC_PROBE_BLOCKS;
    }
    if (coh_ok) {
        const int64_t ntiles = (int64_t)((g.nr + g.r0 % cth + cth - 1) / cth) * ctpr;
        const unsigned cblocks = (unsigned)((ntiles + GBC_WAVES - 1) / GBC_WAVES);
        if (probe) {
            auto pk = key64 ? gbm_coherent_kernel<true, true> : gbm_coherent_kernel<false, true>;
            MHS_HIP(hipFuncSetAttribute((const void *)pk, hipFuncAttributeMaxDynamicSharedMemorySize, (int)gbc_lds_bytes()));
            hipLaunchKernelGGL(pk, dim3(GBC_PROBE_BLOCKS), dim3(1024), gbc_lds_bytes(), st, m->lut, tt.lut_cls, tt.sorted, tt.sorted_off,
                               m->n_trees_padded, m->init_f, m->p, s, g, ctpr, w, acc, out, probe, 1, tt.axis_rank, tt.axis_ncol);
        }
        auto ck = key64 ? gbm_coherent_kernel<true> : gbm_coherent_kernel<false>;
        MHS_HIP(hipFuncSetAttribute((const void *)ck, hipFuncAttributeMaxDynamicSharedMemorySize, (int)gbc_lds_bytes()));
        hipLaunchKernelGGL(ck, dim3(cblocks), dim3(1024), gbc_lds_bytes(), st, m->lut, tt.lut_cls, tt.sorted, tt.sorted_off,
                           m->n_trees_padded, m->init_f, m->p, s, g, ctpr, w, acc, out, probe, 1, tt.axis_rank, tt.axis_ncol);
        if (!probe) return launch_gbm_na(m, s, g, w, acc, out, st, total);
    }
    if (rt_ok) {
        const int64_t ntiles = (int64_t)g.nr * tpr;
        const unsigned rblocks = (unsigned)((ntiles + 3) / 4);
        auto rk = key64 ? gbm_lutreg_rt_kernel<true> : gbm_lutreg_rt_kernel<false>;
        MHS_HIP(hipFuncSetAttribute((const void *)rk, hipFuncAttributeMaxDynamicSharedMemorySize, (int)lut_bytes));
        hipLaunchKernelGGL(rk, dim3(rblocks), dim3(256), lut_bytes, st, tt.lut_rt, (const u64x8 *)tt.lut_rt_meta, tt.sorted, tt.sorted_off,
                           m->n_trees_padded, m->init_f, m->p, s, g, tpr, w, acc, out, (const int *)probe);
        return launch_gbm_na(m, s, g, w, acc, out, st, total);
    }
    const size_t bytes = in_regs ? lut_bytes : (size_t)m->p * 256 * LUT_R * sizeof(float) + lut_bytes;
    auto kern = in_regs ? (m->lut_S == 5 ? (key64 ? gbm_lutreg_kernel<5, true> : gbm_lutreg_kernel<5, false>)
                                         : (key64 ? gbm_lutreg_kernel<6, true> : gbm_lutreg_kernel<6, false>))
                        : (m->lut_S == 5 ? gbm_lut_kernel<5> : gbm_lut_kernel<6>);
    MHS_HIP(hipFuncSetAttribute((const void *)kern, hipFuncAttributeMaxDynamicSharedMemorySize, (int)bytes));
    hipLaunchKernelGGL(kern, dim3(blocks), dim3(256), bytes, st, m->lut, tt.lut_meta, tt.sorted, key64, tt.sorted_off,
                       m->n_trees_padded, m->init_f, m->p, s, g, w, acc, out);
    return launch_gbm_na(m, s, g, w, acc, out, st, total);
}


static int launch_model(const mhs_model *m, const StackDev &s, const PredGeom &g, double weight,
                        int accumulate, double *out, hipStream_t st, const mhs_grid *grid = nullptr) {
    const int64_t total = (int64_t)g.nr * g.nc;
    if (total == 0) return MHS_OK;
    const unsigned blocks = (unsigned)((total + 255) / 256);
    switch (m->kind) {
        case K_LM:
            hipLaunchKernelGGL(lm_kernel, dim3(blocks), dim3(256), 0, st, m->dpar, m->p, s, g, weight, accumulate, out);
            break;
        case K_NNET: {
#define CALL_NNET(P) launch_nnet<P>(m, s, g, weight, accumulate, out, st, blocks)
            MHS_DISPATCH_P(m->p, CALL_NNET)
#undef CALL_NNET
            break;
        }
        case K_EARTH:
            hipLaunchKernelGGL(earth_kernel, dim3(blocks), dim3(256), 0, st, m->dpar, m->dpar + m->n0,
                               m->ipar, m->ipar + m->n0 + 1, m->ipar + m->n0 + 1 + m->n1, m->n0, m->p, s, g,
                               weight, accumulate, out);
            break;
        case K_SVR: {
#define CALL_SVR(P) if (int rc = launch_svr<P>(m, s, g, weight, accumulate, out, st, total)) return rc
            MHS_DISPATCH_P(m->p, CALL_SVR)
#undef CALL_SVR
            break;
        }
        case K_GBM:
            if (gbm_lut_applies(m, s, grid)) {
                if (int rc = launch_gbm_lut(m, s, g, *grid, weight, accumulate, out, st, total)) return rc;
            } else if (int rc = launch_trees<true, false>(m, s, g, weight, accumulate, out, st, total)) return rc;
            break;
        case K_RF: {
            bool launched = false;
            if (int rc = launch_forest(m, s, g, grid, weight, accumulate, out, st, total, &launched)) return rc;
            if (!launched) if (int rc = launch_trees<false, false>(m, s, g, weight, accumulate, out, st, total)) return rc;
            break;
        }
        default:
            set_error("predict: unknown model kind %d", m->kind);
            return MHS_ERR_INVALID;
    }
    MHS_HIP(hipGetLastError());
    return MHS_OK;
}

template <int P>
static void launch_small(const SmallArgs &a, const StackDev &s, const PredGeom &g, int acc, double *out, hipStream_t st, unsigned blocks) {
    hipLaunchKernelGGL((small_members_kernel<P>), dim3(blocks), dim3(256), 0, st, a, s, g, acc, out);
}

int launch_members(const mhs_model *const *models, const double *weights, int n_models, const StackDev &s,
                          const PredGeom &g, int accumulate_first, double *out, hipStream_t st, const mhs_grid *grid) {
    const int64_t total = (int64_t)g.nr * g.nc;
    int k = 0;
    bool masked_done = false;
    int mask_kind = -1;
    for (int want : {K_RF, K_SVR, K_GBM})
        for (int q = 0; q < n_models && mask_kind < 0; ++q)
            if (models[q]->kind == want) mask_kind = want;
    while (k < n_models) {
        const int acc = (k > 0 || accumulate_first) ? 1 : 0;
        int e = k;
        const mhs_model *lm = nullptr, *nn = nullptr, *ea = nullptr;
        if (total > 0 && models[k]->p <= PMAX) {
            if (e < n_models && models[e]->kind == K_LM) lm = models[e++];
            if (e < n_models && models[e]->kind == K_NNET && models[e]->p == models[k]->p) nn = models[e++];
            if (e < n_models && models[e]->kind == K_EARTH && models[e]->p == models[k]->p) ea = models[e++];
        }
        if (e - k >= 2) {
            SmallArgs a{};
            if (lm) { a.lm_coef = lm->dpar; a.w_lm = weights[k]; }
            if (nn) { a.nn_w = nn->dpar; a.nn_H = nn->n0; a.nn_scale = nn->s0; a.nn_shift = nn->s1; a.w_nn = weights[k + (lm ? 1 : 0)]; }
            if (ea) {
                a.ea_coef = ea->dpar; a.ea_cut = ea->dpar + ea->n0; a.ea_tstart = ea->ipar; a.ea_fvar = ea->ipar + ea->n0 + 1;
                a.ea_fdir = ea->ipar + ea->n0 + 1 + ea->n1; a.ea_nterms = ea->n0; a.w_ea = weights[e - 1];
            }
            const unsigned blocks = (unsigned)((total + 255) / 256);
            const int P_ = models[k]->p;
#define CALL_SMALL(P) launch_small<P>(a, s, g, acc, out, st, blocks)
            MHS_DISPATCH_P(P_, CALL_SMALL)
#undef CALL_SMALL
            MHS_HIP(hipGetLastError());
            k = e;
            continue;
        }
        const int kind = models[k]->kind;
        if (!masked_done && ctx().reserved_cus > 0 && grid && total >= (1 << 22) && kind == mask_kind) {
            Context &c = ctx();
            std::lock_guard<std::mutex> lk(mask_mutex());
            if (c.masked_stream) {
                masked_done = true;
                MHS_HIP(hipEventRecord(c.mask_ev0, st));
                MHS_HIP(hipStreamWaitEvent(c.masked_stream, c.mask_ev0, 0));
                if (int rc = launch_model(models[k], s, g, weights[k], acc, out, c.masked_stream, grid)) return rc;
                MHS_HIP(hipEventRecord(c.mask_ev1, c.masked_stream));
                MHS_HIP(hipStreamWaitEvent(st, c.mask_ev1, 0));
                ++k;
                continue;
            }
        }
        if (int rc = launch_model(models[k], s, g, weights[k], acc, out, st, grid)) return rc;
        ++k;
    }
    return MHS_OK;
}

static int make_stack(const mhs_model *m, const mhs_grid *g, const mhs_stack *c, StackDev *s) {
    MHS_REQUIRE(c && c->data, "covariate stack is NULL");
    MHS_REQUIRE(c->n_layers == m->p - 2, "stack has the wrong number of layers for this model (p = layers + 2)");
    MHS_REQUIRE(c->dtype == MHS_F64 || c->dtype == MHS_F32 || c->dtype == MHS_I16, "bad stack dtype");
    MHS_REQUIRE(c->ld >= g->ncol && c->plane_stride >= c->ld * g->nrow, "stack strides smaller than the grid");
    *s = StackDev{c->data, c->n_layers, c->dtype, c->plane_stride, c->ld, c->nodata, !std::isnan(c->nodata), 0};
    return MHS_OK;
}

StackDev rows_stack(const void *buf, int64_t r0, int64_t r1, int n_layers, int dtype, int64_t ld, double nodata) {
    return StackDev{(const char *)buf - (size_t)r0 * ld * dtype_bytes(dtype), n_layers, dtype, (r1 - r0) * ld, ld, nodata, !std::isnan(nodata), 0};
}

static void points_stack(const double *X_dev, int p, int64_t n, StackDev *s, PredGeom *pg) {
    *s = StackDev{X_dev, p, MHS_F64, n, n, NAN, 0, 1};
    *pg = PredGeom{0, 0, 1, 1, 0, 0, 1, (int)n, n};
}

int scale_window(double *out, int64_t nr, int64_t nc, int64_t ld, double wt_total, hipStream_t st) {
    if (nr * nc == 0) return MHS_OK;
    hipLaunchKernelGGL(scale_window_kernel, dim3((unsigned)((nr * nc + 255) / 256)), dim3(256), 0, st, out, (int)nr, (int)nc, ld, wt_total);
    MHS_HIP(hipGetLastError());
    return MHS_OK;
}

int make_geom(const mhs_grid *g, int64_t r0, int64_t r1, int64_t c0, int64_t c1, int64_t ld, PredGeom *pg) {
    MHS_REQUIRE(g && g->nrow > 0 && g->ncol > 0 && g->xres > 0 && g->yres > 0, "bad grid geometry");
    MHS_REQUIRE(0 <= r0 && r0 <= r1 && r1 <= g->nrow && 0 <= c0 && c0 <= c1 && c1 <= g->ncol, "window outside the grid");
    MHS_REQUIRE(ld >= c1 - c0, "ld smaller than the window width");
    MHS_REQUIRE((r1 - r0) * (c1 - c0) < (1LL << 40) && r1 - r0 < (1LL << 31) && c1 - c0 < (1LL << 31), "window too large");
    pg->xmin = g->xmin; pg->ymax = g->ymax; pg->xres = g->xres; pg->yres = g->yres;
    pg->r0 = r0; pg->c0 = c0; pg->nr = (int)(r1 - r0); pg->nc = (int)(c1 - c0); pg->ld_out = ld;
    return MHS_OK;
}

int members_rows_dev(const mhs_model *const *models, const double *weights, int n_models, int accumulate, int scale, double wt_total,
                     const mhs_grid *g, const void *buf, int64_t buf_r0, int64_t buf_r1, int n_layers, int dtype, int64_t ld,
                     double nodata, int64_t b0, int64_t b1, double *out_dev, int64_t ld_out, hipStream_t st) {
    MHS_REQUIRE(models && weights && n_models >= 0 && g && buf && out_dev, "bad ensemble arguments");
    MHS_REQUIRE(wt_total != 0.0 && !std::isnan(wt_total), "wt_total must be non-zero");
    MHS_REQUIRE(dtype == MHS_F64 || dtype == MHS_F32 || dtype == MHS_I16, "bad stack dtype");
    MHS_REQUIRE(buf_r0 <= b0 && b0 <= b1 && b1 <= buf_r1, "rows outside the buffer");
    for (int k = 0; k < n_models; ++k)
        MHS_REQUIRE(models[k] && n_layers == models[k]->p - 2, "stack has the wrong number of layers for a model");
    if (b1 == b0) return MHS_OK;
    PredGeom pg;
    if (int rc = make_geom(g, b0, b1, 0, g->ncol, ld_out, &pg)) return rc;
    const StackDev sd = rows_stack(buf, buf_r0, buf_r1, n_layers, dtype, ld, nodata);
    if (n_models > 0) if (int rc = launch_members(models, weights, n_models, sd, pg, accumulate, out_dev, st, g)) return rc;
    return scale ? scale_window(out_dev, b1 - b0, g->ncol, ld_out, wt_total, st) : MHS_OK;
}

int ensemble_band_dev(const mhs_model *const *models, const double *weights, int n_models, double wt_total, const mhs_grid *g,
                      const void *band_data, int n_layers, int dtype, int64_t ld, double nodata, int64_t b0, int64_t b1,
                      double *out_dev, int64_t ld_out, hipStream_t st) {
    MHS_REQUIRE(n_models >= 1, "bad ensemble arguments");
    return members_rows_dev(models, weights, n_models, 0, 1, wt_total, g, band_data, b0, b1, n_layers, dtype, ld, nodata, b0, b1, out_dev,
                            ld_out, st);
}

}

using namespace mhs;

extern "C" {

int mhs_predict_dev(const mhs_model *m, const mhs_grid *g, const mhs_stack *covars, int64_t r0,
                    int64_t r1, int64_t c0, int64_t c1, double weight, int accumulate, double *out_dev,
                    int64_t ld, void *stream) {
    if (int rc = require_ready()) return rc;
    MHS_REQUIRE(m && out_dev, "NULL argument");
    PredGeom pg;
    StackDev s;
    if (int rc = make_geom(g, r0, r1, c0, c1, ld, &pg)) return rc;
    if (int rc = make_stack(m, g, covars, &s)) return rc;
    return launch_model(m, s, pg, weight, accumulate, out_dev, pick_stream(stream), g);
}

int mhs_members_predict_dev(const mhs_model *const *models, const double *weights, int n_models, const mhs_grid *g,
                            const mhs_stack *covars, int64_t r0, int64_t r1, int64_t c0, int64_t c1, int accumulate,
                            double *out_dev, int64_t ld, void *stream) {
    if (int rc = require_ready()) return rc;
    MHS_REQUIRE(models && weights && n_models >= 1 && out_dev, "bad arguments");
    PredGeom pg;
    StackDev s;
    if (int rc = make_geom(g, r0, r1, c0, c1, ld, &pg)) return rc;
    for (int k = 0; k < n_models; ++k) {
        MHS_REQUIRE(models[k] != nullptr, "NULL model");
        if (int rc = make_stack(models[k], g, covars, &s)) return rc;
    }
    return launch_members(models, weights, n_models, s, pg, accumulate, out_dev, pick_stream(stream), g);
}

int mhs_ensemble_predict_dev(const mhs_model *const *models, const double *weights, int n_models,
                             double wt_total, const mhs_grid *g, const mhs_stack *covars, int64_t r0,
                             int64_t r1, int64_t c0, int64_t c1, double *out_dev, int64_t ld, void *stream) {
    if (int rc = require_ready()) return rc;
    MHS_REQUIRE(models && weights && n_models >= 1 && out_dev, "bad ensemble arguments");
    MHS_REQUIRE(wt_total != 0.0 && !std::isnan(wt_total), "wt_total must be non-zero");
    if (int rc = mhs_members_predict_dev(models, weights, n_models, g, covars, r0, r1, c0, c1, 0, out_dev, ld, stream)) return rc;
    return scale_window(out_dev, r1 - r0, c1 - c0, ld, wt_total, pick_stream(stream));
}

int mhs_predict_points(const mhs_model *m, const double *X, int64_t n, double *out_host) {
    if (int rc = require_ready()) return rc;
    MHS_REQUIRE(m && out_host && (X || n == 0) && n >= 0 && n < (1LL << 31), "bad arguments");
    if (n == 0) return MHS_OK;
    hipStream_t s = ctx().stream;
    DevBuf<double> dx, dout;
    MHS_HIP(dx.alloc((size_t)n * m->p));
    MHS_HIP(dout.alloc((size_t)n));
    MHS_HIP(hipMemcpyAsync(dx.p, X, sizeof(double) * (size_t)n * m->p, hipMemcpyHostToDevice, s));
    PredGeom pg;
    StackDev sd;
    points_stack(dx.p, m->p, n, &sd, &pg);
    if (int rc = launch_model(m, sd, pg, 1.0, 0, dout.p, s)) return rc;
    MHS_HIP(hipMemcpyAsync(out_host, dout.p, sizeof(double) * (size_t)n, hipMemcpyDeviceToHost, s));
    MHS_HIP(hipStreamSynchronize(s));
    return MHS_OK;
}

int mhs_gbm_probe_last(const mhs_model *m, int64_t *cost, int64_t *count) {
    if (int rc = require_ready()) return rc;
    MHS_REQUIRE(m && cost && count, "NULL argument");
    *cost = 0; *count = 0;
    if (m->kind != K_GBM || !m->gbm_probe || m->gbm_probe_next.load() == 0) return MHS_OK;
    int h[2 * GBC_PROBE_BLOCKS];
    MHS_HIP(hipDeviceSynchronize());
    MHS_HIP(hipMemcpy(h, m->gbm_probe + (size_t)((m->gbm_probe_next.load() - 1) % GBC_PROBE_SLOTS) * 2 * GBC_PROBE_BLOCKS, sizeof(h),
                      hipMemcpyDeviceToHost));
    for (int b = 0; b < GBC_PROBE_BLOCKS; ++b) { *cost += h[2 * b]; *count += h[2 * b + 1]; }
    return MHS_OK;
}

int mhs_gbm_staged_points(const mhs_model *m, const double *X, int64_t n, int step, double *out_host) {
    if (int rc = require_ready()) return rc;
    MHS_REQUIRE(m && X && out_host && n >= 1 && n < (1LL << 31) && step >= 1, "bad arguments");
    MHS_REQUIRE(m->kind == K_GBM, "not a gbm model");
    const int stages = m->n_trees / step;
    if (stages == 0) return MHS_OK;
    hipStream_t s = ctx().stream;
    DevBuf<double> dx, dout;
    MHS_HIP(dx.alloc((size_t)n * m->p));
    MHS_HIP(dout.alloc((size_t)n * stages));
    MHS_HIP(hipMemcpyAsync(dx.p, X, sizeof(double) * (size_t)n * m->p, hipMemcpyHostToDevice, s));
    hipLaunchKernelGGL(gbm_staged_points_kernel, dim3((unsigned)((n + 255) / 256)), dim3(256), 0, s, m->nodes, m->tree_off,
                       m->n_trees, m->init_f, dx.p, n, step, dout.p);
    MHS_HIP(hipGetLastError());
    MHS_HIP(hipMemcpyAsync(out_host, dout.p, sizeof(double) * (size_t)n * stages, hipMemcpyDeviceToHost, s));
    MHS_HIP(hipStreamSynchronize(s));
    return MHS_OK;
}

int mhs_residual_points(const mhs_model *const *models, const double *weights, int n_models, double wt_total,
                        const double *X, const double *resp, int64_t n, double *out_host) {
    if (int rc = require_ready()) return rc;
    MHS_REQUIRE(models && weights && X && resp && out_host && n_models >= 1 && n >= 1 && n < (1LL << 31), "bad arguments");
    MHS_REQUIRE(n_models <= 8, "at most 8 members");
    const int p = models[0]->p;
    for (int k = 0; k < n_models; ++k) MHS_REQUIRE(models[k] && models[k]->p == p, "models disagree on the number of predictors");
    hipStream_t s = ctx().stream;
    Context &c = ctx();
    const size_t need = (size_t)n * ((size_t)p + (size_t)n_models + 2);
    if (need > c.points_arena_cap) {
        if (c.points_arena) { (void)hipStreamSynchronize(s); (void)hipFree(c.points_arena); c.points_arena = nullptr; c.points_arena_cap = 0; }
        MHS_HIP(hipMalloc((void **)&c.points_arena, need * sizeof(double)));
        c.points_arena_cap = need;
    }
    double *dx = c.points_arena, *dpred = dx + (size_t)n * p, *dresp = dpred + (size_t)n * n_models, *dout = dresp + n;
    MHS_HIP(hipMemcpyAsync(dx, X, sizeof(double) * (size_t)n * p, hipMemcpyHostToDevice, s));
    MHS_HIP(hipMemcpyAsync(dresp, resp, sizeof(double) * (size_t)n, hipMemcpyHostToDevice, s));
    PredGeom pg;
    StackDev sd;
    points_stack(dx, p, n, &sd, &pg);
    for (int k = 0; k < n_models; ++k)
        if (int rc = launch_model(models[k], sd, pg, 1.0, 0, dpred + (size_t)k * n, s)) return rc;
    ResidualArgs ra;
    for (int k = 0; k < 8; ++k) ra.w[k] = k < n_models ? weights[k] : 0.0;
    hipLaunchKernelGGL(residual_points_kernel, dim3((unsigned)((n + 255) / 256)), dim3(256), 0, s, dpred, dresp, n, n_models, ra,
                       wt_total, dout);
    MHS_HIP(hipGetLastError());
    MHS_HIP(hipMemcpyAsync(out_host, dout, sizeof(double) * (size_t)n, hipMemcpyDeviceToHost, s));
    MHS_HIP(hipStreamSynchronize(s));
    return MHS_OK;
}

int mhs_scale_add_dev(const double *a, double divisor, const double *b, double *out, int64_t n, void *stream) {
    if (int rc = require_ready()) return rc;
    MHS_REQUIRE(a && out && n >= 0, "bad arguments");
    if (n == 0) return MHS_OK;
    hipLaunchKernelGGL(scale_add_kernel, dim3((unsigned)((n + 255) / 256)), dim3(256), 0, pick_stream(stream), a, divisor, b, out, n);
    MHS_HIP(hipGetLastError());
    return MHS_OK;
}

}
```

Measured before the change: 451.8 Mcells/s.

## Replace SVR row-tile inner loop with hand-scheduled inline assembly for P=5

For the P=5 SVR resident kernel, the support-vector accumulation loop is replaced by hand-written GCN assembly. It software-pipelines scalar loads of SV records, LDS reads of the per-SV offset and the exp-table lookups across the three columns, and uses fixed registers with clamp modifiers. The goal is to hide LDS and scalar-load latency and cut instruction overhead beyond what the compiler schedules. The cost is a large fragile asm block with hardcoded registers, a trap check that the LDS table sits at address 0, and an environment fallback to the C++ loop.

```diff
diff --git a/machisplin_amd/csrc/ensemble.hip b/machisplin_amd/csrc/ensemble.hip
--- a/machisplin_amd/csrc/ensemble.hip
+++ b/machisplin_amd/csrc/ensemble.hip
@@ -252,12 +252,13 @@
 }
 
 __device__ __attribute__((noinline)) double svr_rt_exp_call(double z) { return exp(z); }
-template <int P, int R, bool TAB2, bool EXPCALL>
+template <int P, int R, bool TAB2, bool EXPCALL, bool HAND = false>
 __device__ __forceinline__ void svr_rt_tile(const double *__restrict__ svp, int nsv, int stride, int npos,
                                             const double *__restrict__ xcs, const double *etab, double *aw, double sigma, double b,
                                             double amax, double y_center, double y_scale, const StackDev &s, const PredGeom &g,
                                             int row, int tcol, int lane, double weight, int accumulate, double *__restrict__ out) {
     constexpr int CH = 128;
+    static_assert(!HAND || (P == 5 && R == 3 && TAB2), "svr_rt_loop5*.inc are written for P = 5, R = 3 and the 64 KB table");
     double x[R][P], q[R], acc[R], accn[R];
     bool na[R], ok[R];
     int col[R];
@@ -285,7 +286,7 @@
     const bool fold = __builtin_amdgcn_readfirstlane((int)(qhi - qlo <= 0.5)) != 0;
     const double S = fold ? qhi : 0.0;
     double magic = 0.0, c1 = 0.0;
-    if constexpr (TAB2) rt_exp_consts(magic, c1);
+    if constexpr (TAB2 && !HAND) rt_exp_consts(magic, c1);
     auto sum_range = [&](int v0, int v1, double (&a)[R], auto folded) {
         constexpr bool FOLD = decltype(folded)::value;
         auto pair = [&](const double *sp, const double ap) {
@@ -306,6 +307,41 @@
                 aw[e] = fma(sp[P - 1], xlat, sp[P]) + S;
             }
             __builtin_amdgcn_wave_barrier();
+            if constexpr (HAND) {
+                int nt = (n - 1) >> 2;
+                const int rem = n - 4 * nt;
+                unsigned ca = (unsigned)(uintptr_t)(__attribute__((address_space(3))) double *)aw;
+                const double *rec = svp + (int64_t)vb * stride;
+                const int rec_bytes = stride * (int)sizeof(double);
+                const double NK = -EXP_RANGE * EXP_SCALE, NMAGIC = -RT_EXP_MAGIC, C2 = 0.5 / (EXP_SCALE * EXP_SCALE);
+                constexpr unsigned long long MGB = __builtin_bit_cast(unsigned long long, RT_EXP_MAGIC),
+                                             C1B = __builtin_bit_cast(unsigned long long, RT_EXP_C1);
+#define MHS_SVR_LOOP_CLOBBERS                                                                                                       \
+    "memory", "scc", "s84", "s85", "s86", "s87", "s88", "s89", "s90", "s91", "s92", "s93", "s94", "s95", "s96", "s97", "s98",     \
+        "s99", "s100", "v102", "v103", "v104", "v105", "v106", "v107", "v108", "v109", "v110", "v111", "v112", "v113", "v114",       \
+        "v115", "v116", "v117", "v118", "v119", "v120", "v121", "v122", "v123", "v124", "v125", "v126", "v127"
+#define MHS_SVR_LOOP_X                                                                                                              \
+    [x00] "v"(x[0][0]), [x01] "v"(x[0][1]), [x02] "v"(x[0][2]), [x03] "v"(x[0][3]), [x10] "v"(x[1][0]), [x11] "v"(x[1][1]),        \
+        [x12] "v"(x[1][2]), [x13] "v"(x[1][3]), [x20] "v"(x[2][0]), [x21] "v"(x[2][1]), [x22] "v"(x[2][2]), [x23] "v"(x[2][3]),    \
+        [mglo] "i"((unsigned)MGB), [mghi] "i"((unsigned)(MGB >> 32)), [c1lo] "i"((unsigned)C1B),                    \
+        [c1hi] "i"((unsigned)(C1B >> 32)), [rem] "s"(rem), [sp] "s"(rec), [st] "s"(rec_bytes), [nk] "s"(NK), [nm] "s"(NMAGIC),     \
+        [c2] "s"(C2)
+                if constexpr (FOLD)
+                    asm volatile(
+#include "svr_rt_loop5.inc"
+                        : [a0] "+v"(a[0]), [a1] "+v"(a[1]), [a2] "+v"(a[2]), [ca] "+v"(ca), [nt] "+s"(nt)
+                        : MHS_SVR_LOOP_X
+                        : MHS_SVR_LOOP_CLOBBERS);
+                else
+                    asm volatile(
+#include "svr_rt_loop5q.inc"
+                        : [a0] "+v"(a[0]), [a1] "+v"(a[1]), [a2] "+v"(a[2]), [ca] "+v"(ca), [nt] "+s"(nt)
+                        : MHS_SVR_LOOP_X, [q0] "v"(q[0]), [q1] "v"(q[1]), [q2] "v"(q[2])
+                        : MHS_SVR_LOOP_CLOBBERS);
+#undef MHS_SVR_LOOP_X
+#undef MHS_SVR_LOOP_CLOBBERS
+                continue;
+            }
             const double *sp = svp + (int64_t)vb * stride;
             const double *ar = aw;
             int e = 0;
@@ -333,13 +369,13 @@
         }
 }
 
-template <int P, int R, bool TAB2>
+template <int P, int R, bool TAB2, bool HAND>
 __device__ __forceinline__ void svr_rt_run(int64_t tile, const double *__restrict__ svp, int nsv, int stride, int npos,
                                            const double *__restrict__ xcs, const double *etab, double *aw, double sigma, double b,
                                            double amax, double y_center, double y_scale, const StackDev &s, const PredGeom &g,
                                            int tiles_per_row, int lane, double weight, int accumulate, double *__restrict__ out) {
     const int row = (int)(tile / tiles_per_row), tcol = (int)(tile - (int64_t)row * tiles_per_row) * (64 * R);
-    svr_rt_tile<P, R, TAB2, true>(svp, nsv, stride, npos, xcs, etab, aw, sigma, b, amax, y_center, y_scale, s, g, row, tcol, lane, weight,
+    svr_rt_tile<P, R, TAB2, true, HAND>(svp, nsv, stride, npos, xcs, etab, aw, sigma, b, amax, y_center, y_scale, s, g, row, tcol, lane, weight,
                                   accumulate, out);
 }
 template <int NW, bool TAB2>
@@ -385,12 +421,20 @@
     (void)g0; (void)g1; (void)g2; (void)g3; (void)g4; (void)g5; (void)g6; (void)g7; (void)g8;
     (void)s0; (void)s1; (void)s2; (void)s3; (void)s4; (void)s5; (void)s6; (void)s7;
 }
-template <int P, int R, int NW, bool TAB2, int WPS>
+template <int NW, bool TAB2>
+struct alignas(16) SvrRtLds {
+    double etab[TAB2 ? EXP_TAB2_N : EXP_TAB_N];
+    double aw[NW][128];
+};
+template <int P, int R, int NW, bool TAB2, int WPS, bool HAND>
 __global__ __launch_bounds__(64 * NW, WPS) void svr_rt_resident_kernel(const double *__restrict__ svp, const double *__restrict__ xcs,
                                                                   const double *__restrict__ gtab, double *__restrict__ out,
                                                                   unsigned long long *__restrict__ pool, SvrRtScalars sc) {
-    __shared__ double etab[TAB2 ? EXP_TAB2_N : EXP_TAB_N];
-    __shared__ double aw[NW][128];
+    __shared__ SvrRtLds<NW, TAB2> lds;
+    double *const etab = lds.etab;
+    auto &aw = lds.aw;
+    if constexpr (HAND)
+        if ((unsigned)(uintptr_t)(__attribute__((address_space(3))) double *)lds.etab != 0u) __builtin_trap();
     svr_rt_stage<NW, TAB2>(etab, gtab);
     __syncthreads();
     const int wave = threadIdx.x >> 6, lane = threadIdx.x & 63;
@@ -406,7 +450,7 @@
         const PredGeom g = {k->g.xmin, k->g.ymax, k->g.xres, k->g.yres, k->g.r0, k->g.c0, k->g.nr, k->g.nc, k->g.ld_out};
         if (tile >= (int64_t)g.nr * k->tiles_per_row) return;
         const StackDev s = {k->s.data, k->s.C, k->s.dtype, k->s.plane_stride, k->s.ld, k->s.nodata, k->s.has_nodata, k->s.all_from_planes};
-        svr_rt_run<P, R, TAB2>(tile, svp, k->nsv, k->stride, k->npos, xcs, etab, aw[wave], k->sigma, k->b, k->amax,
+        svr_rt_run<P, R, TAB2, HAND>(tile, svp, k->nsv, k->stride, k->npos, xcs, etab, aw[wave], k->sigma, k->b, k->amax,
                                k->y_center, k->y_scale, s, g, k->tiles_per_row, lane, k->weight, k->accumulate, out);
     }
 }
@@ -1133,6 +1177,7 @@
 constexpr bool svr_rt_tab2(int P) { return P <= 5; }
 constexpr int svr_rt_waves_per_simd(int P) { return P <= 5 ? 4 : 3; }
 constexpr int svr_rt_waves(int P) { return svr_rt_tab2(P) ? 16 : 4; }
+constexpr bool svr_rt_hand(int P) { return P == 5; }
 
 static std::mutex svr_pool_mu[MAX_SLOTS];
 static int svr_pool_take(Context &c, hipStream_t st, int *idx, unsigned long long **counter) {
@@ -1158,10 +1203,13 @@
         constexpr int NW = svr_rt_waves(P);
         const int64_t covering = (ntiles + NW - 1) / NW;
         if constexpr (svr_rt_tab2(P)) {
-            auto kern = svr_rt_resident_kernel<P, R, NW, true, svr_rt_waves_per_simd(P)>;
+            const bool hand = svr_rt_hand(P) && !getenv("MHS_SVR_CXX_LOOP");
+            auto kern = svr_rt_resident_kernel<P, R, NW, true, svr_rt_waves_per_simd(P), false>;
+            if constexpr (svr_rt_hand(P))
+                if (hand) kern = svr_rt_resident_kernel<P, R, NW, true, svr_rt_waves_per_simd(P), true>;
             Context &c = ctx();
             std::lock_guard<std::mutex> lk(svr_pool_mu[current_slot()]);
-            int &per_cu = c.svr_rt_blocks_per_cu[P];
+            int &per_cu = c.svr_rt_blocks_per_cu[hand ? 0 : P];
             if (per_cu == 0) {
                 int n = 0;
                 MHS_HIP(hipOccupancyMaxActiveBlocksPerMultiprocessor(&n, (const void *)kern, 64 * NW, 0));
diff --git a/machisplin_amd/csrc/svr_rt_loop5.inc b/machisplin_amd/csrc/svr_rt_loop5.inc
--- /dev/null
+++ b/machisplin_amd/csrc/svr_rt_loop5.inc
@@ -0,0 +1,426 @@
+"v_mov_b32_e32 v124, %[mglo]\n\t"
+"v_mov_b32_e32 v125, %[mghi]\n\t"
+"v_mov_b32_e32 v126, %[c1lo]\n\t"
+"v_mov_b32_e32 v127, %[c1hi]\n\t"
+"s_mov_b32 s100, 0\n\t"
+"s_cmp_eq_u32 %[nt], 0\n\t"
+"s_cbranch_scc1 3f\n\t"
+"s_load_dwordx8 s[84:91], %[sp], s100\n\t"
+"s_add_u32 s100, s100, %[st]\n\t"
+"ds_read_b64 v[102:103], %[ca]\n\t"
+"s_waitcnt lgkmcnt(0)\n\t"
+"s_load_dwordx8 s[92:99], %[sp], s100\n\t"
+"s_add_u32 s100, s100, %[st]\n\t"
+"ds_read_b64 v[104:105], %[ca] offset:8\n\t"
+"v_fma_f64 v[106:107], s[84:85], %[x00], v[102:103]\n\t"
+"v_fmac_f64_e32 v[106:107], s[86:87], %[x01]\n\t"
+"v_fmac_f64_e32 v[106:107], s[88:89], %[x02]\n\t"
+"v_fma_f64 v[106:107], s[90:91], %[x03], v[106:107] clamp\n\t"
+"v_fma_f64 v[108:109], %[nk], v[106:107], v[124:125]\n\t"
+"v_add_f64 v[110:111], v[108:109], %[nm]\n\t"
+"v_lshlrev_b16 v109, 3, v108\n\t"
+"v_fma_f64 v[110:111], v[106:107], %[nk], -v[110:111]\n\t"
+"ds_read_b64 v[106:107], v109\n\t"
+"v_fma_f64 v[112:113], s[84:85], %[x10], v[102:103]\n\t"
+"v_fmac_f64_e32 v[112:113], s[86:87], %[x11]\n\t"
+"v_fmac_f64_e32 v[112:113], s[88:89], %[x12]\n\t"
+"v_fma_f64 v[112:113], s[90:91], %[x13], v[112:113] clamp\n\t"
+"v_fma_f64 v[114:115], %[nk], v[112:113], v[124:125]\n\t"
+"v_add_f64 v[116:117], v[114:115], %[nm]\n\t"
+"v_lshlrev_b16 v115, 3, v114\n\t"
+"v_fma_f64 v[116:117], v[112:113], %[nk], -v[116:117]\n\t"
+"ds_read_b64 v[112:113], v115\n\t"
+"s_branch 2f\n\t"
+"1:\n\t"
+"s_load_dwordx8 s[92:99], %[sp], s100\n\t"
+"s_add_u32 s100, s100, %[st]\n\t"
+"ds_read_b64 v[104:105], %[ca] offset:8\n\t"
+"v_fma_f64 v[106:107], s[84:85], %[x00], v[102:103]\n\t"
+"v_fmac_f64_e32 v[106:107], s[86:87], %[x01]\n\t"
+"v_fmac_f64_e32 v[106:107], s[88:89], %[x02]\n\t"
+"v_fma_f64 v[106:107], s[90:91], %[x03], v[106:107] clamp\n\t"
+"v_fma_f64 v[108:109], %[nk], v[106:107], v[124:125]\n\t"
+"v_add_f64 v[110:111], v[108:109], %[nm]\n\t"
+"v_lshlrev_b16 v109, 3, v108\n\t"
+"v_fma_f64 v[110:111], v[106:107], %[nk], -v[110:111]\n\t"
+"ds_read_b64 v[106:107], v109\n\t"
+"s_waitcnt lgkmcnt(3)\n\t"
+"v_lshl_add_u32 v113, v114, 8, v113\n\t"
+"v_fma_f64 v[114:115], %[c2], v[116:117], v[126:127]\n\t"
+"v_fma_f64 v[114:115], v[114:115], v[116:117], 1.0\n\t"
+"v_fmac_f64_e32 %[a1], v[112:113], v[114:115]\n\t"
+"v_fma_f64 v[112:113], s[84:85], %[x10], v[102:103]\n\t"
+"v_fmac_f64_e32 v[112:113], s[86:87], %[x11]\n\t"
+"v_fmac_f64_e32 v[112:113], s[88:89], %[x12]\n\t"
+"v_fma_f64 v[112:113], s[90:91], %[x13], v[112:113] clamp\n\t"
+"v_fma_f64 v[114:115], %[nk], v[112:113], v[124:125]\n\t"
+"v_add_f64 v[116:117], v[114:115], %[nm]\n\t"
+"v_lshlrev_b16 v115, 3, v114\n\t"
+"v_fma_f64 v[116:117], v[112:113], %[nk], -v[116:117]\n\t"
+"ds_read_b64 v[112:113], v115\n\t"
+"s_waitcnt lgkmcnt(3)\n\t"
+"v_lshl_add_u32 v119, v120, 8, v119\n\t"
+"v_fma_f64 v[120:121], %[c2], v[122:123], v[126:127]\n\t"
+"v_fma_f64 v[120:121], v[120:121], v[122:123], 1.0\n\t"
+"v_fmac_f64_e32 %[a2], v[118:119], v[120:121]\n\t"
+"2:\n\t"
+"v_fma_f64 v[118:119], s[84:85], %[x20], v[102:103]\n\t"
+"v_fmac_f64_e32 v[118:119], s[86:87], %[x21]\n\t"
+"v_fmac_f64_e32 v[118:119], s[88:89], %[x22]\n\t"
+"v_fma_f64 v[118:119], s[90:91], %[x23], v[118:119] clamp\n\t"
+"v_fma_f64 v[120:121], %[nk], v[118:119], v[124:125]\n\t"
+"v_add_f64 v[122:123], v[120:121], %[nm]\n\t"
+"v_lshlrev_b16 v121, 3, v120\n\t"
+"v_fma_f64 v[122:123], v[118:119], %[nk], -v[122:123]\n\t"
+"s_waitcnt lgkmcnt(0)\n\t"
+"ds_read_b64 v[118:119], v121\n\t"
+"s_waitcnt lgkmcnt(2)\n\t"
+"v_lshl_add_u32 v107, v108, 8, v107\n\t"
+"v_fma_f64 v[108:109], %[c2], v[110:111], v[126:127]\n\t"
+"v_fma_f64 v[108:109], v[108:109], v[110:111], 1.0\n\t"
+"v_fmac_f64_e32 %[a0], v[106:107], v[108:109]\n\t"
+"s_load_dwordx8 s[84:91], %[sp], s100\n\t"
+"s_add_u32 s100, s100, %[st]\n\t"
+"ds_read_b64 v[102:103], %[ca] offset:16\n\t"
+"v_fma_f64 v[106:107], s[92:93], %[x00], v[104:105]\n\t"
+"v_fmac_f64_e32 v[106:107], s[94:95], %[x01]\n\t"
+"v_fmac_f64_e32 v[106:107], s[96:97], %[x02]\n\t"
+"v_fma_f64 v[106:107], s[98:99], %[x03], v[106:107] clamp\n\t"
+"v_fma_f64 v[108:109], %[nk], v[106:107], v[124:125]\n\t"
+"v_add_f64 v[110:111], v[108:109], %[nm]\n\t"
+"v_lshlrev_b16 v109, 3, v108\n\t"
+"v_fma_f64 v[110:111], v[106:107], %[nk], -v[110:111]\n\t"
+"ds_read_b64 v[106:107], v109\n\t"
+"s_waitcnt lgkmcnt(3)\n\t"
+"v_lshl_add_u32 v113, v114, 8, v113\n\t"
+"v_fma_f64 v[114:115], %[c2], v[116:117], v[126:127]\n\t"
+"v_fma_f64 v[114:115], v[114:115], v[116:117], 1.0\n\t"
+"v_fmac_f64_e32 %[a1], v[112:113], v[114:115]\n\t"
+"v_fma_f64 v[112:113], s[92:93], %[x10], v[104:105]\n\t"
+"v_fmac_f64_e32 v[112:113], s[94:95], %[x11]\n\t"
+"v_fmac_f64_e32 v[112:113], s[96:97], %[x12]\n\t"
+"v_fma_f64 v[112:113], s[98:99], %[x13], v[112:113] clamp\n\t"
+"v_fma_f64 v[114:115], %[nk], v[112:113], v[124:125]\n\t"
+"v_add_f64 v[116:117], v[114:115], %[nm]\n\t"
+"v_lshlrev_b16 v115, 3, v114\n\t"
+"v_fma_f64 v[116:117], v[112:113], %[nk], -v[116:117]\n\t"
+"ds_read_b64 v[112:113], v115\n\t"
+"s_waitcnt lgkmcnt(3)\n\t"
+"v_lshl_add_u32 v119, v120, 8, v119\n\t"
+"v_fma_f64 v[120:121], %[c2], v[122:123], v[126:127]\n\t"
+"v_fma_f64 v[120:121], v[120:121], v[122:123], 1.0\n\t"
+"v_fmac_f64_e32 %[a2], v[118:119], v[120:121]\n\t"
+"v_fma_f64 v[118:119], s[92:93], %[x20], v[104:105]\n\t"
+"v_fmac_f64_e32 v[118:119], s[94:95], %[x21]\n\t"
+"v_fmac_f64_e32 v[118:119], s[96:97], %[x22]\n\t"
+"v_fma_f64 v[118:119], s[98:99], %[x23], v[118:119] clamp\n\t"
+"v_fma_f64 v[120:121], %[nk], v[118:119], v[124:125]\n\t"
+"v_add_f64 v[122:123], v[120:121], %[nm]\n\t"
+"v_lshlrev_b16 v121, 3, v120\n\t"
+"v_fma_f64 v[122:123], v[118:119], %[nk], -v[122:123]\n\t"
+"s_waitcnt lgkmcnt(0)\n\t"
+"ds_read_b64 v[118:119], v121\n\t"
+"s_waitcnt lgkmcnt(2)\n\t"
+"v_lshl_add_u32 v107, v108, 8, v107\n\t"
+"v_fma_f64 v[108:109], %[c2], v[110:111], v[126:127]\n\t"
+"v_fma_f64 v[108:109], v[108:109], v[110:111], 1.0\n\t"
+"v_fmac_f64_e32 %[a0], v[106:107], v[108:109]\n\t"
+"s_load_dwordx8 s[92:99], %[sp], s100\n\t"
+"s_add_u32 s100, s100, %[st]\n\t"
+"ds_read_b64 v[104:105], %[ca] offset:24\n\t"
+"v_fma_f64 v[106:107], s[84:85], %[x00], v[102:103]\n\t"
+"v_fmac_f64_e32 v[106:107], s[86:87], %[x01]\n\t"
+"v_fmac_f64_e32 v[106:107], s[88:89], %[x02]\n\t"
+"v_fma_f64 v[106:107], s[90:91], %[x03], v[106:107] clamp\n\t"
+"v_fma_f64 v[108:109], %[nk], v[106:107], v[124:125]\n\t"
+"v_add_f64 v[110:111], v[108:109], %[nm]\n\t"
+"v_lshlrev_b16 v109, 3, v108\n\t"
+"v_fma_f64 v[110:111], v[106:107], %[nk], -v[110:111]\n\t"
+"ds_read_b64 v[106:107], v109\n\t"
+"s_waitcnt lgkmcnt(3)\n\t"
+"v_lshl_add_u32 v113, v114, 8, v113\n\t"
+"v_fma_f64 v[114:115], %[c2], v[116:117], v[126:127]\n\t"
+"v_fma_f64 v[114:115], v[114:115], v[116:117], 1.0\n\t"
+"v_fmac_f64_e32 %[a1], v[112:113], v[114:115]\n\t"
+"v_fma_f64 v[112:113], s[84:85], %[x10], v[102:103]\n\t"
+"v_fmac_f64_e32 v[112:113], s[86:87], %[x11]\n\t"
+"v_fmac_f64_e32 v[112:113], s[88:89], %[x12]\n\t"
+"v_fma_f64 v[112:113], s[90:91], %[x13], v[112:113] clamp\n\t"
+"v_fma_f64 v[114:115], %[nk], v[112:113], v[124:125]\n\t"
+"v_add_f64 v[116:117], v[114:115], %[nm]\n\t"
+"v_lshlrev_b16 v115, 3, v114\n\t"
+"v_fma_f64 v[116:117], v[112:113], %[nk], -v[116:117]\n\t"
+"ds_read_b64 v[112:113], v115\n\t"
+"s_waitcnt lgkmcnt(3)\n\t"
+"v_lshl_add_u32 v119, v120, 8, v119\n\t"
+"v_fma_f64 v[120:121], %[c2], v[122:123], v[126:127]\n\t"
+"v_fma_f64 v[120:121], v[120:121], v[122:123], 1.0\n\t"
+"v_fmac_f64_e32 %[a2], v[118:119], v[120:121]\n\t"
+"v_fma_f64 v[118:119], s[84:85], %[x20], v[102:103]\n\t"
+"v_fmac_f64_e32 v[118:119], s[86:87], %[x21]\n\t"
+"v_fmac_f64_e32 v[118:119], s[88:89], %[x22]\n\t"
+"v_fma_f64 v[118:119], s[90:91], %[x23], v[118:119] clamp\n\t"
+"v_fma_f64 v[120:121], %[nk], v[118:119], v[124:125]\n\t"
+"v_add_f64 v[122:123], v[120:121], %[nm]\n\t"
+"v_lshlrev_b16 v121, 3, v120\n\t"
+"v_fma_f64 v[122:123], v[118:119], %[nk], -v[122:123]\n\t"
+"s_waitcnt lgkmcnt(0)\n\t"
+"ds_read_b64 v[118:119], v121\n\t"
+"s_waitcnt lgkmcnt(2)\n\t"
+"v_lshl_add_u32 v107, v108, 8, v107\n\t"
+"v_fma_f64 v[108:109], %[c2], v[110:111], v[126:127]\n\t"
+"v_fma_f64 v[108:109], v[108:109], v[110:111], 1.0\n\t"
+"v_fmac_f64_e32 %[a0], v[106:107], v[108:109]\n\t"
+"s_load_dwordx8 s[84:91], %[sp], s100\n\t"
+"s_add_u32 s100, s100, %[st]\n\t"
+"ds_read_b64 v[102:103], %[ca] offset:32\n\t"
+"v_fma_f64 v[106:107], s[92:93], %[x00], v[104:105]\n\t"
+"v_fmac_f64_e32 v[106:107], s[94:95], %[x01]\n\t"
+"v_fmac_f64_e32 v[106:107], s[96:97], %[x02]\n\t"
+"v_fma_f64 v[106:107], s[98:99], %[x03], v[106:107] clamp\n\t"
+"v_fma_f64 v[108:109], %[nk], v[106:107], v[124:125]\n\t"
+"v_add_f64 v[110:111], v[108:109], %[nm]\n\t"
+"v_lshlrev_b16 v109, 3, v108\n\t"
+"v_fma_f64 v[110:111], v[106:107], %[nk], -v[110:111]\n\t"
+"ds_read_b64 v[106:107], v109\n\t"
+"s_waitcnt lgkmcnt(3)\n\t"
+"v_lshl_add_u32 v113, v114, 8, v113\n\t"
+"v_fma_f64 v[114:115], %[c2], v[116:117], v[126:127]\n\t"
+"v_fma_f64 v[114:115], v[114:115], v[116:117], 1.0\n\t"
+"v_fmac_f64_e32 %[a1], v[112:113], v[114:115]\n\t"
+"v_fma_f64 v[112:113], s[92:93], %[x10], v[104:105]\n\t"
+"v_fmac_f64_e32 v[112:113], s[94:95], %[x11]\n\t"
+"v_fmac_f64_e32 v[112:113], s[96:97], %[x12]\n\t"
+"v_fma_f64 v[112:113], s[98:99], %[x13], v[112:113] clamp\n\t"
+"v_fma_f64 v[114:115], %[nk], v[112:113], v[124:125]\n\t"
+"v_add_f64 v[116:117], v[114:115], %[nm]\n\t"
+"v_lshlrev_b16 v115, 3, v114\n\t"
+"v_fma_f64 v[116:117], v[112:113], %[nk], -v[116:117]\n\t"
+"ds_read_b64 v[112:113], v115\n\t"
+"s_waitcnt lgkmcnt(3)\n\t"
+"v_lshl_add_u32 v119, v120, 8, v119\n\t"
+"v_fma_f64 v[120:121], %[c2], v[122:123], v[126:127]\n\t"
+"v_fma_f64 v[120:121], v[120:121], v[122:123], 1.0\n\t"
+"v_fmac_f64_e32 %[a2], v[118:119], v[120:121]\n\t"
+"v_fma_f64 v[118:119], s[92:93], %[x20], v[104:105]\n\t"
+"v_fmac_f64_e32 v[118:119], s[94:95], %[x21]\n\t"
+"v_fmac_f64_e32 v[118:119], s[96:97], %[x22]\n\t"
+"v_fma_f64 v[118:119], s[98:99], %[x23], v[118:119] clamp\n\t"
+"v_fma_f64 v[120:121], %[nk], v[118:119], v[124:125]\n\t"
+"v_add_f64 v[122:123], v[120:121], %[nm]\n\t"
+"v_lshlrev_b16 v121, 3, v120\n\t"
+"v_fma_f64 v[122:123], v[118:119], %[nk], -v[122:123]\n\t"
+"s_waitcnt lgkmcnt(0)\n\t"
+"ds_read_b64 v[118:119], v121\n\t"
+"s_waitcnt lgkmcnt(2)\n\t"
+"v_lshl_add_u32 v107, v108, 8, v107\n\t"
+"v_fma_f64 v[108:109], %[c2], v[110:111], v[126:127]\n\t"
+"v_fma_f64 v[108:109], v[108:109], v[110:111], 1.0\n\t"
+"v_fmac_f64_e32 %[a0], v[106:107], v[108:109]\n\t"
+"v_add_u32_e32 %[ca], 32, %[ca]\n\t"
+"s_sub_u32 %[nt], %[nt], 1\n\t"
+"s_cmp_lg_u32 %[nt], 0\n\t"
+"s_cbranch_scc1 1b\n\t"
+"s_waitcnt lgkmcnt(1)\n\t"
+"v_lshl_add_u32 v113, v114, 8, v113\n\t"
+"v_fma_f64 v[114:115], %[c2], v[116:117], v[126:127]\n\t"
+"v_fma_f64 v[114:115], v[114:115], v[116:117], 1.0\n\t"
+"v_fmac_f64_e32 %[a1], v[112:113], v[114:115]\n\t"
+"s_waitcnt lgkmcnt(0)\n\t"
+"v_lshl_add_u32 v119, v120, 8, v119\n\t"
+"v_fma_f64 v[120:121], %[c2], v[122:123], v[126:127]\n\t"
+"v_fma_f64 v[120:121], v[120:121], v[122:123], 1.0\n\t"
+"v_fmac_f64_e32 %[a2], v[118:119], v[120:121]\n\t"
+"s_sub_u32 s100, s100, %[st]\n\t"
+"3:\n\t"
+"s_load_dwordx8 s[84:91], %[sp], s100\n\t"
+"s_add_u32 s100, s100, %[st]\n\t"
+"ds_read_b64 v[102:103], %[ca] offset:0\n\t"
+"s_waitcnt lgkmcnt(0)\n\t"
+"v_fma_f64 v[106:107], s[84:85], %[x00], v[102:103]\n\t"
+"v_fmac_f64_e32 v[106:107], s[86:87], %[x01]\n\t"
+"v_fmac_f64_e32 v[106:107], s[88:89], %[x02]\n\t"
+"v_fma_f64 v[106:107], s[90:91], %[x03], v[106:107] clamp\n\t"
+"v_fma_f64 v[108:109], %[nk], v[106:107], v[124:125]\n\t"
+"v_add_f64 v[110:111], v[108:109], %[nm]\n\t"
+"v_lshlrev_b16 v109, 3, v108\n\t"
+"v_fma_f64 v[110:111], v[106:107], %[nk], -v[110:111]\n\t"
+"ds_read_b64 v[106:107], v109\n\t"
+"v_fma_f64 v[112:113], s[84:85], %[x10], v[102:103]\n\t"
+"v_fmac_f64_e32 v[112:113], s[86:87], %[x11]\n\t"
+"v_fmac_f64_e32 v[112:113], s[88:89], %[x12]\n\t"
+"v_fma_f64 v[112:113], s[90:91], %[x13], v[112:113] clamp\n\t"
+"v_fma_f64 v[114:115], %[nk], v[112:113], v[124:125]\n\t"
+"v_add_f64 v[116:117], v[114:115], %[nm]\n\t"
+"v_lshlrev_b16 v115, 3, v114\n\t"
+"v_fma_f64 v[116:117], v[112:113], %[nk], -v[116:117]\n\t"
+"ds_read_b64 v[112:113], v115\n\t"
+"s_waitcnt lgkmcnt(1)\n\t"
+"v_lshl_add_u32 v107, v108, 8, v107\n\t"
+"v_fma_f64 v[108:109], %[c2], v[110:111], v[126:127]\n\t"
+"v_fma_f64 v[108:109], v[108:109], v[110:111], 1.0\n\t"
+"v_fmac_f64_e32 %[a0], v[106:107], v[108:109]\n\t"
+"v_fma_f64 v[118:119], s[84:85], %[x20], v[102:103]\n\t"
+"v_fmac_f64_e32 v[118:119], s[86:87], %[x21]\n\t"
+"v_fmac_f64_e32 v[118:119], s[88:89], %[x22]\n\t"
+"v_fma_f64 v[118:119], s[90:91], %[x23], v[118:119] clamp\n\t"
+"v_fma_f64 v[120:121], %[nk], v[118:119], v[124:125]\n\t"
+"v_add_f64 v[122:123], v[120:121], %[nm]\n\t"
+"v_lshlrev_b16 v121, 3, v120\n\t"
+"v_fma_f64 v[122:123], v[118:119], %[nk], -v[122:123]\n\t"
+"ds_read_b64 v[118:119], v121\n\t"
+"s_waitcnt lgkmcnt(1)\n\t"
+"v_lshl_add_u32 v113, v114, 8, v113\n\t"
+"v_fma_f64 v[114:115], %[c2], v[116:117], v[126:127]\n\t"
+"v_fma_f64 v[114:115], v[114:115], v[116:117], 1.0\n\t"
+"v_fmac_f64_e32 %[a1], v[112:113], v[114:115]\n\t"
+"s_waitcnt lgkmcnt(0)\n\t"
+"v_lshl_add_u32 v119, v120, 8, v119\n\t"
+"v_fma_f64 v[120:121], %[c2], v[122:123], v[126:127]\n\t"
+"v_fma_f64 v[120:121], v[120:121], v[122:123], 1.0\n\t"
+"v_fmac_f64_e32 %[a2], v[118:119], v[120:121]\n\t"
+"s_cmp_eq_u32 %[rem], 1\n\t"
+"s_cbranch_scc1 9f\n\t"
+"s_load_dwordx8 s[84:91], %[sp], s100\n\t"
+"s_add_u32 s100, s100, %[st]\n\t"
+"ds_read_b64 v[102:103], %[ca] offset:8\n\t"
+"s_waitcnt lgkmcnt(0)\n\t"
+"v_fma_f64 v[106:107], s[84:85], %[x00], v[102:103]\n\t"
+"v_fmac_f64_e32 v[106:107], s[86:87], %[x01]\n\t"
+"v_fmac_f64_e32 v[106:107], s[88:89], %[x02]\n\t"
+"v_fma_f64 v[106:107], s[90:91], %[x03], v[106:107] clamp\n\t"
+"v_fma_f64 v[108:109], %[nk], v[106:107], v[124:125]\n\t"
+"v_add_f64 v[110:111], v[108:109], %[nm]\n\t"
+"v_lshlrev_b16 v109, 3, v108\n\t"
+"v_fma_f64 v[110:111], v[106:107], %[nk], -v[110:111]\n\t"
+"ds_read_b64 v[106:107], v109\n\t"
+"v_fma_f64 v[112:113], s[84:85], %[x10], v[102:103]\n\t"
+"v_fmac_f64_e32 v[112:113], s[86:87], %[x11]\n\t"
+"v_fmac_f64_e32 v[112:113], s[88:89], %[x12]\n\t"
+"v_fma_f64 v[112:113], s[90:91], %[x13], v[112:113] clamp\n\t"
+"v_fma_f64 v[114:115], %[nk], v[112:113], v[124:125]\n\t"
+"v_add_f64 v[116:117], v[114:115], %[nm]\n\t"
+"v_lshlrev_b16 v115, 3, v114\n\t"
+"v_fma_f64 v[116:117], v[112:113], %[nk], -v[116:117]\n\t"
+"ds_read_b64 v[112:113], v115\n\t"
+"s_waitcnt lgkmcnt(1)\n\t"
+"v_lshl_add_u32 v107, v108, 8, v107\n\t"
+"v_fma_f64 v[108:109], %[c2], v[110:111], v[126:127]\n\t"
+"v_fma_f64 v[108:109], v[108:109], v[110:111], 1.0\n\t"
+"v_fmac_f64_e32 %[a0], v[106:107], v[108:109]\n\t"
+"v_fma_f64 v[118:119], s[84:85], %[x20], v[102:103]\n\t"
+"v_fmac_f64_e32 v[118:119], s[86:87], %[x21]\n\t"
+"v_fmac_f64_e32 v[118:119], s[88:89], %[x22]\n\t"
+"v_fma_f64 v[118:119], s[90:91], %[x23], v[118:119] clamp\n\t"
+"v_fma_f64 v[120:121], %[nk], v[118:119], v[124:125]\n\t"
+"v_add_f64 v[122:123], v[120:121], %[nm]\n\t"
+"v_lshlrev_b16 v121, 3, v120\n\t"
+"v_fma_f64 v[122:123], v[118:119], %[nk], -v[122:123]\n\t"
+"ds_read_b64 v[118:119], v121\n\t"
+"s_waitcnt lgkmcnt(1)\n\t"
+"v_lshl_add_u32 v113, v114, 8, v113\n\t"
+"v_fma_f64 v[114:115], %[c2], v[116:117], v[126:127]\n\t"
+"v_fma_f64 v[114:115], v[114:115], v[116:117], 1.0\n\t"
+"v_fmac_f64_e32 %[a1], v[112:113], v[114:115]\n\t"
+"s_waitcnt lgkmcnt(0)\n\t"
+"v_lshl_add_u32 v119, v120, 8, v119\n\t"
+"v_fma_f64 v[120:121], %[c2], v[122:123], v[126:127]\n\t"
+"v_fma_f64 v[120:121], v[120:121], v[122:123], 1.0\n\t"
+"v_fmac_f64_e32 %[a2], v[118:119], v[120:121]\n\t"
+"s_cmp_eq_u32 %[rem], 2\n\t"
+"s_cbranch_scc1 9f\n\t"
+"s_load_dwordx8 s[84:91], %[sp], s100\n\t"
+"s_add_u32 s100, s100, %[st]\n\t"
+"ds_read_b64 v[102:103], %[ca] offset:16\n\t"
+"s_waitcnt lgkmcnt(0)\n\t"
+"v_fma_f64 v[106:107], s[84:85], %[x00], v[102:103]\n\t"
+"v_fmac_f64_e32 v[106:107], s[86:87], %[x01]\n\t"
+"v_fmac_f64_e32 v[106:107], s[88:89], %[x02]\n\t"
+"v_fma_f64 v[106:107], s[90:91], %[x03], v[106:107] clamp\n\t"
+"v_fma_f64 v[108:109], %[nk], v[106:107], v[124:125]\n\t"
+"v_add_f64 v[110:111], v[108:109], %[nm]\n\t"
+"v_lshlrev_b16 v109, 3, v108\n\t"
+"v_fma_f64 v[110:111], v[106:107], %[nk], -v[110:111]\n\t"
+"ds_read_b64 v[106:107], v109\n\t"
+"v_fma_f64 v[112:113], s[84:85], %[x10], v[102:103]\n\t"
+"v_fmac_f64_e32 v[112:113], s[86:87], %[x11]\n\t"
+"v_fmac_f64_e32 v[112:113], s[88:89], %[x12]\n\t"
+"v_fma_f64 v[112:113], s[90:91], %[x13], v[112:113] clamp\n\t"
+"v_fma_f64 v[114:115], %[nk], v[112:113], v[124:125]\n\t"
+"v_add_f64 v[116:117], v[114:115], %[nm]\n\t"
+"v_lshlrev_b16 v115, 3, v114\n\t"
+"v_fma_f64 v[116:117], v[112:113], %[nk], -v[116:117]\n\t"
+"ds_read_b64 v[112:113], v115\n\t"
+"s_waitcnt lgkmcnt(1)\n\t"
+"v_lshl_add_u32 v107, v108, 8, v107\n\t"
+"v_fma_f64 v[108:109], %[c2], v[110:111], v[126:127]\n\t"
+"v_fma_f64 v[108:109], v[108:109], v[110:111], 1.0\n\t"
+"v_fmac_f64_e32 %[a0], v[106:107], v[108:109]\n\t"
+"v_fma_f64 v[118:119], s[84:85], %[x20], v[102:103]\n\t"
+"v_fmac_f64_e32 v[118:119], s[86:87], %[x21]\n\t"
+"v_fmac_f64_e32 v[118:119], s[88:89], %[x22]\n\t"
+"v_fma_f64 v[118:119], s[90:91], %[x23], v[118:119] clamp\n\t"
+"v_fma_f64 v[120:121], %[nk], v[118:119], v[124:125]\n\t"
+"v_add_f64 v[122:123], v[120:121], %[nm]\n\t"
+"v_lshlrev_b16 v121, 3, v120\n\t"
+"v_fma_f64 v[122:123], v[118:119], %[nk], -v[122:123]\n\t"
+"ds_read_b64 v[118:119], v121\n\t"
+"s_waitcnt lgkmcnt(1)\n\t"
+"v_lshl_add_u32 v113, v114, 8, v113\n\t"
+"v_fma_f64 v[114:115], %[c2], v[116:117], v[126:127]\n\t"
+"v_fma_f64 v[114:115], v[114:115], v[116:117], 1.0\n\t"
+"v_fmac_f64_e32 %[a1], v[112:113], v[114:115]\n\t"
+"s_waitcnt lgkmcnt(0)\n\t"
+"v_lshl_add_u32 v119, v120, 8, v119\n\t"
+"v_fma_f64 v[120:121], %[c2], v[122:123], v[126:127]\n\t"
+"v_fma_f64 v[120:121], v[120:121], v[122:123], 1.0\n\t"
+"v_fmac_f64_e32 %[a2], v[118:119], v[120:121]\n\t"
+"s_cmp_eq_u32 %[rem], 3\n\t"
+"s_cbranch_scc1 9f\n\t"
+"s_load_dwordx8 s[84:91], %[sp], s100\n\t"
+"s_add_u32 s100, s100, %[st]\n\t"
+"ds_read_b64 v[102:103], %[ca] offset:24\n\t"
+"s_waitcnt lgkmcnt(0)\n\t"
+"v_fma_f64 v[106:107], s[84:85], %[x00], v[102:103]\n\t"
+"v_fmac_f64_e32 v[106:107], s[86:87], %[x01]\n\t"
+"v_fmac_f64_e32 v[106:107], s[88:89], %[x02]\n\t"
+"v_fma_f64 v[106:107], s[90:91], %[x03], v[106:107] clamp\n\t"
+"v_fma_f64 v[108:109], %[nk], v[106:107], v[124:125]\n\t"
+"v_add_f64 v[110:111], v[108:109], %[nm]\n\t"
+"v_lshlrev_b16 v109, 3, v108\n\t"
+"v_fma_f64 v[110:111], v[106:107], %[nk], -v[110:111]\n\t"
+"ds_read_b64 v[106:107], v109\n\t"
+"v_fma_f64 v[112:113], s[84:85], %[x10], v[102:103]\n\t"
+"v_fmac_f64_e32 v[112:113], s[86:87], %[x11]\n\t"
+"v_fmac_f64_e32 v[112:113], s[88:89], %[x12]\n\t"
+"v_fma_f64 v[112:113], s[90:91], %[x13], v[112:113] clamp\n\t"
+"v_fma_f64 v[114:115], %[nk], v[112:113], v[124:125]\n\t"
+"v_add_f64 v[116:117], v[114:115], %[nm]\n\t"
+"v_lshlrev_b16 v115, 3, v114\n\t"
+"v_fma_f64 v[116:117], v[112:113], %[nk], -v[116:117]\n\t"
+"ds_read_b64 v[112:113], v115\n\t"
+"s_waitcnt lgkmcnt(1)\n\t"
+"v_lshl_add_u32 v107, v108, 8, v107\n\t"
+"v_fma_f64 v[108:109], %[c2], v[110:111], v[126:127]\n\t"
+"v_fma_f64 v[108:109], v[108:109], v[110:111], 1.0\n\t"
+"v_fmac_f64_e32 %[a0], v[106:107], v[108:109]\n\t"
+"v_fma_f64 v[118:119], s[84:85], %[x20], v[102:103]\n\t"
+"v_fmac_f64_e32 v[118:119], s[86:87], %[x21]\n\t"
+"v_fmac_f64_e32 v[118:119], s[88:89], %[x22]\n\t"
+"v_fma_f64 v[118:119], s[90:91], %[x23], v[118:119] clamp\n\t"
+"v_fma_f64 v[120:121], %[nk], v[118:119], v[124:125]\n\t"
+"v_add_f64 v[122:123], v[120:121], %[nm]\n\t"
+"v_lshlrev_b16 v121, 3, v120\n\t"
+"v_fma_f64 v[122:123], v[118:119], %[nk], -v[122:123]\n\t"
+"ds_read_b64 v[118:119], v121\n\t"
+"s_waitcnt lgkmcnt(1)\n\t"
+"v_lshl_add_u32 v113, v114, 8, v113\n\t"
+"v_fma_f64 v[114:115], %[c2], v[116:117], v[126:127]\n\t"
+"v_fma_f64 v[114:115], v[114:115], v[116:117], 1.0\n\t"
+"v_fmac_f64_e32 %[a1], v[112:113], v[114:115]\n\t"
+"s_waitcnt lgkmcnt(0)\n\t"
+"v_lshl_add_u32 v119, v120, 8, v119\n\t"
+"v_fma_f64 v[120:121], %[c2], v[122:123], v[126:127]\n\t"
+"v_fma_f64 v[120:121], v[120:121], v[122:123], 1.0\n\t"
+"v_fmac_f64_e32 %[a2], v[118:119], v[120:121]\n\t"
+"9:\n\t"
diff --git a/machisplin_amd/csrc/svr_rt_loop5q.inc b/machisplin_amd/csrc/svr_rt_loop5q.inc
--- /dev/null
+++ b/machisplin_amd/csrc/svr_rt_loop5q.inc
@@ -0,0 +1,452 @@
+"v_mov_b32_e32 v124, %[mglo]\n\t"
+"v_mov_b32_e32 v125, %[mghi]\n\t"
+"v_mov_b32_e32 v126, %[c1lo]\n\t"
+"v_mov_b32_e32 v127, %[c1hi]\n\t"
+"s_mov_b32 s100, 0\n\t"
+"s_cmp_eq_u32 %[nt], 0\n\t"
+"s_cbranch_scc1 3f\n\t"
+"s_load_dwordx8 s[84:91], %[sp], s100\n\t"
+"s_add_u32 s100, s100, %[st]\n\t"
+"ds_read_b64 v[102:103], %[ca]\n\t"
+"s_waitcnt lgkmcnt(0)\n\t"
+"s_load_dwordx8 s[92:99], %[sp], s100\n\t"
+"s_add_u32 s100, s100, %[st]\n\t"
+"ds_read_b64 v[104:105], %[ca] offset:8\n\t"
+"v_add_f64 v[106:107], %[q0], v[102:103]\n\t"
+"v_fmac_f64_e32 v[106:107], s[84:85], %[x00]\n\t"
+"v_fmac_f64_e32 v[106:107], s[86:87], %[x01]\n\t"
+"v_fmac_f64_e32 v[106:107], s[88:89], %[x02]\n\t"
+"v_fma_f64 v[106:107], s[90:91], %[x03], v[106:107] clamp\n\t"
+"v_fma_f64 v[108:109], %[nk], v[106:107], v[124:125]\n\t"
+"v_add_f64 v[110:111], v[108:109], %[nm]\n\t"
+"v_lshlrev_b16 v109, 3, v108\n\t"
+"v_fma_f64 v[110:111], v[106:107], %[nk], -v[110:111]\n\t"
+"ds_read_b64 v[106:107], v109\n\t"
+"v_add_f64 v[112:113], %[q1], v[102:103]\n\t"
+"v_fmac_f64_e32 v[112:113], s[84:85], %[x10]\n\t"
+"v_fmac_f64_e32 v[112:113], s[86:87], %[x11]\n\t"
+"v_fmac_f64_e32 v[112:113], s[88:89], %[x12]\n\t"
+"v_fma_f64 v[112:113], s[90:91], %[x13], v[112:113] clamp\n\t"
+"v_fma_f64 v[114:115], %[nk], v[112:113], v[124:125]\n\t"
+"v_add_f64 v[116:117], v[114:115], %[nm]\n\t"
+"v_lshlrev_b16 v115, 3, v114\n\t"
+"v_fma_f64 v[116:117], v[112:113], %[nk], -v[116:117]\n\t"
+"ds_read_b64 v[112:113], v115\n\t"
+"s_branch 2f\n\t"
+"1:\n\t"
+"s_load_dwordx8 s[92:99], %[sp], s100\n\t"
+"s_add_u32 s100, s100, %[st]\n\t"
+"ds_read_b64 v[104:105], %[ca] offset:8\n\t"
+"v_add_f64 v[106:107], %[q0], v[102:103]\n\t"
+"v_fmac_f64_e32 v[106:107], s[84:85], %[x00]\n\t"
+"v_fmac_f64_e32 v[106:107], s[86:87], %[x01]\n\t"
+"v_fmac_f64_e32 v[106:107], s[88:89], %[x02]\n\t"
+"v_fma_f64 v[106:107], s[90:91], %[x03], v[106:107] clamp\n\t"
+"v_fma_f64 v[108:109], %[nk], v[106:107], v[124:125]\n\t"
+"v_add_f64 v[110:111], v[108:109], %[nm]\n\t"
+"v_lshlrev_b16 v109, 3, v108\n\t"
+"v_fma_f64 v[110:111], v[106:107], %[nk], -v[110:111]\n\t"
+"ds_read_b64 v[106:107], v109\n\t"
+"s_waitcnt lgkmcnt(3)\n\t"
+"v_lshl_add_u32 v113, v114, 8, v113\n\t"
+"v_fma_f64 v[114:115], %[c2], v[116:117], v[126:127]\n\t"
+"v_fma_f64 v[114:115], v[114:115], v[116:117], 1.0\n\t"
+"v_fmac_f64_e32 %[a1], v[112:113], v[114:115]\n\t"
+"v_add_f64 v[112:113], %[q1], v[102:103]\n\t"
+"v_fmac_f64_e32 v[112:113], s[84:85], %[x10]\n\t"
+"v_fmac_f64_e32 v[112:113], s[86:87], %[x11]\n\t"
+"v_fmac_f64_e32 v[112:113], s[88:89], %[x12]\n\t"
+"v_fma_f64 v[112:113], s[90:91], %[x13], v[112:113] clamp\n\t"
+"v_fma_f64 v[114:115], %[nk], v[112:113], v[124:125]\n\t"
+"v_add_f64 v[116:117], v[114:115], %[nm]\n\t"
+"v_lshlrev_b16 v115, 3, v114\n\t"
+"v_fma_f64 v[116:117], v[112:113], %[nk], -v[116:117]\n\t"
+"ds_read_b64 v[112:113], v115\n\t"
+"s_waitcnt lgkmcnt(3)\n\t"
+"v_lshl_add_u32 v119, v120, 8, v119\n\t"
+"v_fma_f64 v[120:121], %[c2], v[122:123], v[126:127]\n\t"
+"v_fma_f64 v[120:121], v[120:121], v[122:123], 1.0\n\t"
+"v_fmac_f64_e32 %[a2], v[118:119], v[120:121]\n\t"
+"2:\n\t"
+"v_add_f64 v[118:119], %[q2], v[102:103]\n\t"
+"v_fmac_f64_e32 v[118:119], s[84:85], %[x20]\n\t"
+"v_fmac_f64_e32 v[118:119], s[86:87], %[x21]\n\t"
+"v_fmac_f64_e32 v[118:119], s[88:89], %[x22]\n\t"
+"v_fma_f64 v[118:119], s[90:91], %[x23], v[118:119] clamp\n\t"
+"v_fma_f64 v[120:121], %[nk], v[118:119], v[124:125]\n\t"
+"v_add_f64 v[122:123], v[120:121], %[nm]\n\t"
+"v_lshlrev_b16 v121, 3, v120\n\t"
+"v_fma_f64 v[122:123], v[118:119], %[nk], -v[122:123]\n\t"
+"s_waitcnt lgkmcnt(0)\n\t"
+"ds_read_b64 v[118:119], v121\n\t"
+"s_waitcnt lgkmcnt(2)\n\t"
+"v_lshl_add_u32 v107, v108, 8, v107\n\t"
+"v_fma_f64 v[108:109], %[c2], v[110:111], v[126:127]\n\t"
+"v_fma_f64 v[108:109], v[108:109], v[110:111], 1.0\n\t"
+"v_fmac_f64_e32 %[a0], v[106:107], v[108:109]\n\t"
+"s_load_dwordx8 s[84:91], %[sp], s100\n\t"
+"s_add_u32 s100, s100, %[st]\n\t"
+"ds_read_b64 v[102:103], %[ca] offset:16\n\t"
+"v_add_f64 v[106:107], %[q0], v[104:105]\n\t"
+"v_fmac_f64_e32 v[106:107], s[92:93], %[x00]\n\t"
+"v_fmac_f64_e32 v[106:107], s[94:95], %[x01]\n\t"
+"v_fmac_f64_e32 v[106:107], s[96:97], %[x02]\n\t"
+"v_fma_f64 v[106:107], s[98:99], %[x03], v[106:107] clamp\n\t"
+"v_fma_f64 v[108:109], %[nk], v[106:107], v[124:125]\n\t"
+"v_add_f64 v[110:111], v[108:109], %[nm]\n\t"
+"v_lshlrev_b16 v109, 3, v108\n\t"
+"v_fma_f64 v[110:111], v[106:107], %[nk], -v[110:111]\n\t"
+"ds_read_b64 v[106:107], v109\n\t"
+"s_waitcnt lgkmcnt(3)\n\t"
+"v_lshl_add_u32 v113, v114, 8, v113\n\t"
+"v_fma_f64 v[114:115], %[c2], v[116:117], v[126:127]\n\t"
+"v_fma_f64 v[114:115], v[114:115], v[116:117], 1.0\n\t"
+"v_fmac_f64_e32 %[a1], v[112:113], v[114:115]\n\t"
+"v_add_f64 v[112:113], %[q1], v[104:105]\n\t"
+"v_fmac_f64_e32 v[112:113], s[92:93], %[x10]\n\t"
+"v_fmac_f64_e32 v[112:113], s[94:95], %[x11]\n\t"
+"v_fmac_f64_e32 v[112:113], s[96:97], %[x12]\n\t"
+"v_fma_f64 v[112:113], s[98:99], %[x13], v[112:113] clamp\n\t"
+"v_fma_f64 v[114:115], %[nk], v[112:113], v[124:125]\n\t"
+"v_add_f64 v[116:117], v[114:115], %[nm]\n\t"
+"v_lshlrev_b16 v115, 3, v114\n\t"
+"v_fma_f64 v[116:117], v[112:113], %[nk], -v[116:117]\n\t"
+"ds_read_b64 v[112:113], v115\n\t"
+"s_waitcnt lgkmcnt(3)\n\t"
+"v_lshl_add_u32 v119, v120, 8, v119\n\t"
+"v_fma_f64 v[120:121], %[c2], v[122:123], v[126:127]\n\t"
+"v_fma_f64 v[120:121], v[120:121], v[122:123], 1.0\n\t"
+"v_fmac_f64_e32 %[a2], v[118:119], v[120:121]\n\t"
+"v_add_f64 v[118:119], %[q2], v[104:105]\n\t"
+"v_fmac_f64_e32 v[118:119], s[92:93], %[x20]\n\t"
+"v_fmac_f64_e32 v[118:119], s[94:95], %[x21]\n\t"
+"v_fmac_f64_e32 v[118:119], s[96:97], %[x22]\n\t"
+"v_fma_f64 v[118:119], s[98:99], %[x23], v[118:119] clamp\n\t"
+"v_fma_f64 v[120:121], %[nk], v[118:119], v[124:125]\n\t"
+"v_add_f64 v[122:123], v[120:121], %[nm]\n\t"
+"v_lshlrev_b16 v121, 3, v120\n\t"
+"v_fma_f64 v[122:123], v[118:119], %[nk], -v[122:123]\n\t"
+"s_waitcnt lgkmcnt(0)\n\t"
+"ds_read_b64 v[118:119], v121\n\t"
+"s_waitcnt lgkmcnt(2)\n\t"
+"v_lshl_add_u32 v107, v108, 8, v107\n\t"
+"v_fma_f64 v[108:109], %[c2], v[110:111], v[126:127]\n\t"
+"v_fma_f64 v[108:109], v[108:109], v[110:111], 1.0\n\t"
+"v_fmac_f64_e32 %[a0], v[106:107], v[108:109]\n\t"
+"s_load_dwordx8 s[92:99], %[sp], s100\n\t"
+"s_add_u32 s100, s100, %[st]\n\t"
+"ds_read_b64 v[104:105], %[ca] offset:24\n\t"
+"v_add_f64 v[106:107], %[q0], v[102:103]\n\t"
+"v_fmac_f64_e32 v[106:107], s[84:85], %[x00]\n\t"
+"v_fmac_f64_e32 v[106:107], s[86:87], %[x01]\n\t"
+"v_fmac_f64_e32 v[106:107], s[88:89], %[x02]\n\t"
+"v_fma_f64 v[106:107], s[90:91], %[x03], v[106:107] clamp\n\t"
+"v_fma_f64 v[108:109], %[nk], v[106:107], v[124:125]\n\t"
+"v_add_f64 v[110:111], v[108:109], %[nm]\n\t"
+"v_lshlrev_b16 v109, 3, v108\n\t"
+"v_fma_f64 v[110:111], v[106:107], %[nk], -v[110:111]\n\t"
+"ds_read_b64 v[106:107], v109\n\t"
+"s_waitcnt lgkmcnt(3)\n\t"
+"v_lshl_add_u32 v113, v114, 8, v113\n\t"
+"v_fma_f64 v[114:115], %[c2], v[116:117], v[126:127]\n\t"
+"v_fma_f64 v[114:115], v[114:115], v[116:117], 1.0\n\t"
+"v_fmac_f64_e32 %[a1], v[112:113], v[114:115]\n\t"
+"v_add_f64 v[112:113], %[q1], v[102:103]\n\t"
+"v_fmac_f64_e32 v[112:113], s[84:85], %[x10]\n\t"
+"v_fmac_f64_e32 v[112:113], s[86:87], %[x11]\n\t"
+"v_fmac_f64_e32 v[112:113], s[88:89], %[x12]\n\t"
+"v_fma_f64 v[112:113], s[90:91], %[x13], v[112:113] clamp\n\t"
+"v_fma_f64 v[114:115], %[nk], v[112:113], v[124:125]\n\t"
+"v_add_f64 v[116:117], v[114:115], %[nm]\n\t"
+"v_lshlrev_b16 v115, 3, v114\n\t"
+"v_fma_f64 v[116:117], v[112:113], %[nk], -v[116:117]\n\t"
+"ds_read_b64 v[112:113], v115\n\t"
+"s_waitcnt lgkmcnt(3)\n\t"
+"v_lshl_add_u32 v119, v120, 8, v119\n\t"
+"v_fma_f64 v[120:121], %[c2], v[122:123], v[126:127]\n\t"
+"v_fma_f64 v[120:121], v[120:121], v[122:123], 1.0\n\t"
+"v_fmac_f64_e32 %[a2], v[118:119], v[120:121]\n\t"
+"v_add_f64 v[118:119], %[q2], v[102:103]\n\t"
+"v_fmac_f64_e32 v[118:119], s[84:85], %[x20]\n\t"
+"v_fmac_f64_e32 v[118:119], s[86:87], %[x21]\n\t"
+"v_fmac_f64_e32 v[118:119], s[88:89], %[x22]\n\t"
+"v_fma_f64 v[118:119], s[90:91], %[x23], v[118:119] clamp\n\t"
+"v_fma_f64 v[120:121], %[nk], v[118:119], v[124:125]\n\t"
+"v_add_f64 v[122:123], v[120:121], %[nm]\n\t"
+"v_lshlrev_b16 v121, 3, v120\n\t"
+"v_fma_f64 v[122:123], v[118:119], %[nk], -v[122:123]\n\t"
+"s_waitcnt lgkmcnt(0)\n\t"
+"ds_read_b64 v[118:119], v121\n\t"
+"s_waitcnt lgkmcnt(2)\n\t"
+"v_lshl_add_u32 v107, v108, 8, v107\n\t"
+"v_fma_f64 v[108:109], %[c2], v[110:111], v[126:127]\n\t"
+"v_fma_f64 v[108:109], v[108:109], v[110:111], 1.0\n\t"
+"v_fmac_f64_e32 %[a0], v[106:107], v[108:109]\n\t"
+"s_load_dwordx8 s[84:91], %[sp], s100\n\t"
+"s_add_u32 s100, s100, %[st]\n\t"
+"ds_read_b64 v[102:103], %[ca] offset:32\n\t"
+"v_add_f64 v[106:107], %[q0], v[104:105]\n\t"
+"v_fmac_f64_e32 v[106:107], s[92:93], %[x00]\n\t"
+"v_fmac_f64_e32 v[106:107], s[94:95], %[x01]\n\t"
+"v_fmac_f64_e32 v[106:107], s[96:97], %[x02]\n\t"
+"v_fma_f64 v[106:107], s[98:99], %[x03], v[106:107] clamp\n\t"
+"v_fma_f64 v[108:109], %[nk], v[106:107], v[124:125]\n\t"
+"v_add_f64 v[110:111], v[108:109], %[nm]\n\t"
+"v_lshlrev_b16 v109, 3, v108\n\t"
+"v_fma_f64 v[110:111], v[106:107], %[nk], -v[110:111]\n\t"
+"ds_read_b64 v[106:107], v109\n\t"
+"s_waitcnt lgkmcnt(3)\n\t"
+"v_lshl_add_u32 v113, v114, 8, v113\n\t"
+"v_fma_f64 v[114:115], %[c2], v[116:117], v[126:127]\n\t"
+"v_fma_f64 v[114:115], v[114:115], v[116:117], 1.0\n\t"
+"v_fmac_f64_e32 %[a1], v[112:113], v[114:115]\n\t"
+"v_add_f64 v[112:113], %[q1], v[104:105]\n\t"
+"v_fmac_f64_e32 v[112:113], s[92:93], %[x10]\n\t"
+"v_fmac_f64_e32 v[112:113], s[94:95], %[x11]\n\t"
+"v_fmac_f64_e32 v[112:113], s[96:97], %[x12]\n\t"
+"v_fma_f64 v[112:113], s[98:99], %[x13], v[112:113] clamp\n\t"
+"v_fma_f64 v[114:115], %[nk], v[112:113], v[124:125]\n\t"
+"v_add_f64 v[116:117], v[114:115], %[nm]\n\t"
+"v_lshlrev_b16 v115, 3, v114\n\t"
+"v_fma_f64 v[116:117], v[112:113], %[nk], -v[116:117]\n\t"
+"ds_read_b64 v[112:113], v115\n\t"
+"s_waitcnt lgkmcnt(3)\n\t"
+"v_lshl_add_u32 v119, v120, 8, v119\n\t"
+"v_fma_f64 v[120:121], %[c2], v[122:123], v[126:127]\n\t"
+"v_fma_f64 v[120:121], v[120:121], v[122:123], 1.0\n\t"
+"v_fmac_f64_e32 %[a2], v[118:119], v[120:121]\n\t"
+"v_add_f64 v[118:119], %[q2], v[104:105]\n\t"
+"v_fmac_f64_e32 v[118:119], s[92:93], %[x20]\n\t"
+"v_fmac_f64_e32 v[118:119], s[94:95], %[x21]\n\t"
+"v_fmac_f64_e32 v[118:119], s[96:97], %[x22]\n\t"
+"v_fma_f64 v[118:119], s[98:99], %[x23], v[118:119] clamp\n\t"
+"v_fma_f64 v[120:121], %[nk], v[118:119], v[124:125]\n\t"
+"v_add_f64 v[122:123], v[120:121], %[nm]\n\t"
+"v_lshlrev_b16 v121, 3, v120\n\t"
+"v_fma_f64 v[122:123], v[118:119], %[nk], -v[122:123]\n\t"
+"s_waitcnt lgkmcnt(0)\n\t"
+"ds_read_b64 v[118:119], v121\n\t"
+"s_waitcnt lgkmcnt(2)\n\t"
+"v_lshl_add_u32 v107, v108, 8, v107\n\t"
+"v_fma_f64 v[108:109], %[c2], v[110:111], v[126:127]\n\t"
+"v_fma_f64 v[108:109], v[108:109], v[110:111], 1.0\n\t"
+"v_fmac_f64_e32 %[a0], v[106:107], v[108:109]\n\t"
+"v_add_u32_e32 %[ca], 32, %[ca]\n\t"
+"s_sub_u32 %[nt], %[nt], 1\n\t"
+"s_cmp_lg_u32 %[nt], 0\n\t"
+"s_cbranch_scc1 1b\n\t"
+"s_waitcnt lgkmcnt(1)\n\t"
+"v_lshl_add_u32 v113, v114, 8, v113\n\t"
+"v_fma_f64 v[114:115], %[c2], v[116:117], v[126:127]\n\t"
+"v_fma_f64 v[114:115], v[114:115], v[116:117], 1.0\n\t"
+"v_fmac_f64_e32 %[a1], v[112:113], v[114:115]\n\t"
+"s_waitcnt lgkmcnt(0)\n\t"
+"v_lshl_add_u32 v119, v120, 8, v119\n\t"
+"v_fma_f64 v[120:121], %[c2], v[122:123], v[126:127]\n\t"
+"v_fma_f64 v[120:121], v[120:121], v[122:123], 1.0\n\t"
+"v_fmac_f64_e32 %[a2], v[118:119], v[120:121]\n\t"
+"s_sub_u32 s100, s100, %[st]\n\t"
+"3:\n\t"
+"s_load_dwordx8 s[84:91], %[sp], s100\n\t"
+"s_add_u32 s100, s100, %[st]\n\t"
+"ds_read_b64 v[102:103], %[ca] offset:0\n\t"
+"s_waitcnt lgkmcnt(0)\n\t"
+"v_add_f64 v[106:107], %[q0], v[102:103]\n\t"
+"v_fmac_f64_e32 v[106:107], s[84:85], %[x00]\n\t"
+"v_fmac_f64_e32 v[106:107], s[86:87], %[x01]\n\t"
+"v_fmac_f64_e32 v[106:107], s[88:89], %[x02]\n\t"
+"v_fma_f64 v[106:107], s[90:91], %[x03], v[106:107] clamp\n\t"
+"v_fma_f64 v[108:109], %[nk], v[106:107], v[124:125]\n\t"
+"v_add_f64 v[110:111], v[108:109], %[nm]\n\t"
+"v_lshlrev_b16 v109, 3, v108\n\t"
+"v_fma_f64 v[110:111], v[106:107], %[nk], -v[110:111]\n\t"
+"ds_read_b64 v[106:107], v109\n\t"
+"v_add_f64 v[112:113], %[q1], v[102:103]\n\t"
+"v_fmac_f64_e32 v[112:113], s[84:85], %[x10]\n\t"
+"v_fmac_f64_e32 v[112:113], s[86:87], %[x11]\n\t"
+"v_fmac_f64_e32 v[112:113], s[88:89], %[x12]\n\t"
+"v_fma_f64 v[112:113], s[90:91], %[x13], v[112:113] clamp\n\t"
+"v_fma_f64 v[114:115], %[nk], v[112:113], v[124:125]\n\t"
+"v_add_f64 v[116:117], v[114:115], %[nm]\n\t"
+"v_lshlrev_b16 v115, 3, v114\n\t"
+"v_fma_f64 v[116:117], v[112:113], %[nk], -v[116:117]\n\t"
+"ds_read_b64 v[112:113], v115\n\t"
+"s_waitcnt lgkmcnt(1)\n\t"
+"v_lshl_add_u32 v107, v108, 8, v107\n\t"
+"v_fma_f64 v[108:109], %[c2], v[110:111], v[126:127]\n\t"
+"v_fma_f64 v[108:109], v[108:109], v[110:111], 1.0\n\t"
+"v_fmac_f64_e32 %[a0], v[106:107], v[108:109]\n\t"
+"v_add_f64 v[118:119], %[q2], v[102:103]\n\t"
+"v_fmac_f64_e32 v[118:119], s[84:85], %[x20]\n\t"
+"v_fmac_f64_e32 v[118:119], s[86:87], %[x21]\n\t"
+"v_fmac_f64_e32 v[118:119], s[88:89], %[x22]\n\t"
+"v_fma_f64 v[118:119], s[90:91], %[x23], v[118:119] clamp\n\t"
+"v_fma_f64 v[120:121], %[nk], v[118:119], v[124:125]\n\t"
+"v_add_f64 v[122:123], v[120:121], %[nm]\n\t"
+"v_lshlrev_b16 v121, 3, v120\n\t"
+"v_fma_f64 v[122:123], v[118:119], %[nk], -v[122:123]\n\t"
+"ds_read_b64 v[118:119], v121\n\t"
+"s_waitcnt lgkmcnt(1)\n\t"
+"v_lshl_add_u32 v113, v114, 8, v113\n\t"
+"v_fma_f64 v[114:115], %[c2], v[116:117], v[126:127]\n\t"
+"v_fma_f64 v[114:115], v[114:115], v[116:117], 1.0\n\t"
+"v_fmac_f64_e32 %[a1], v[112:113], v[114:115]\n\t"
+"s_waitcnt lgkmcnt(0)\n\t"
+"v_lshl_add_u32 v119, v120, 8, v119\n\t"
+"v_fma_f64 v[120:121], %[c2], v[122:123], v[126:127]\n\t"
+"v_fma_f64 v[120:121], v[120:121], v[122:123], 1.0\n\t"
+"v_fmac_f64_e32 %[a2], v[118:119], v[120:121]\n\t"
+"s_cmp_eq_u32 %[rem], 1\n\t"
+"s_cbranch_scc1 9f\n\t"
+"s_load_dwordx8 s[84:91], %[sp], s100\n\t"
+"s_add_u32 s100, s100, %[st]\n\t"
+"ds_read_b64 v[102:103], %[ca] offset:8\n\t"
+"s_waitcnt lgkmcnt(0)\n\t"
+"v_add_f64 v[106:107], %[q0], v[102:103]\n\t"
+"v_fmac_f64_e32 v[106:107], s[84:85], %[x00]\n\t"
+"v_fmac_f64_e32 v[106:107], s[86:87], %[x01]\n\t"
+"v_fmac_f64_e32 v[106:107], s[88:89], %[x02]\n\t"
+"v_fma_f64 v[106:107], s[90:91], %[x03], v[106:107] clamp\n\t"
+"v_fma_f64 v[108:109], %[nk], v[106:107], v[124:125]\n\t"
+"v_add_f64 v[110:111], v[108:109], %[nm]\n\t"
+"v_lshlrev_b16 v109, 3, v108\n\t"
+"v_fma_f64 v[110:111], v[106:107], %[nk], -v[110:111]\n\t"
+"ds_read_b64 v[106:107], v109\n\t"
+"v_add_f64 v[112:113], %[q1], v[102:103]\n\t"
+"v_fmac_f64_e32 v[112:113], s[84:85], %[x10]\n\t"
+"v_fmac_f64_e32 v[112:113], s[86:87], %[x11]\n\t"
+"v_fmac_f64_e32 v[112:113], s[88:89], %[x12]\n\t"
+"v_fma_f64 v[112:113], s[90:91], %[x13], v[112:113] clamp\n\t"
+"v_fma_f64 v[114:115], %[nk], v[112:113], v[124:125]\n\t"
+"v_add_f64 v[116:117], v[114:115], %[nm]\n\t"
+"v_lshlrev_b16 v115, 3, v114\n\t"
+"v_fma_f64 v[116:117], v[112:113], %[nk], -v[116:117]\n\t"
+"ds_read_b64 v[112:113], v115\n\t"
+"s_waitcnt lgkmcnt(1)\n\t"
+"v_lshl_add_u32 v107, v108, 8, v107\n\t"
+"v_fma_f64 v[108:109], %[c2], v[110:111], v[126:127]\n\t"
+"v_fma_f64 v[108:109], v[108:109], v[110:111], 1.0\n\t"
+"v_fmac_f64_e32 %[a0], v[106:107], v[108:109]\n\t"
+"v_add_f64 v[118:119], %[q2], v[102:103]\n\t"
+"v_fmac_f64_e32 v[118:119], s[84:85], %[x20]\n\t"
+"v_fmac_f64_e32 v[118:119], s[86:87], %[x21]\n\t"
+"v_fmac_f64_e32 v[118:119], s[88:89], %[x22]\n\t"
+"v_fma_f64 v[118:119], s[90:91], %[x23], v[118:119] clamp\n\t"
+"v_fma_f64 v[120:121], %[nk], v[118:119], v[124:125]\n\t"
+"v_add_f64 v[122:123], v[120:121], %[nm]\n\t"
+"v_lshlrev_b16 v121, 3, v120\n\t"
+"v_fma_f64 v[122:123], v[118:119], %[nk], -v[122:123]\n\t"
+"ds_read_b64 v[118:119], v121\n\t"
+"s_waitcnt lgkmcnt(1)\n\t"
+"v_lshl_add_u32 v113, v114, 8, v113\n\t"
+"v_fma_f64 v[114:115], %[c2], v[116:117], v[126:127]\n\t"
+"v_fma_f64 v[114:115], v[114:115], v[116:117], 1.0\n\t"
+"v_fmac_f64_e32 %[a1], v[112:113], v[114:115]\n\t"
+"s_waitcnt lgkmcnt(0)\n\t"
+"v_lshl_add_u32 v119, v120, 8, v119\n\t"
+"v_fma_f64 v[120:121], %[c2], v[122:123], v[126:127]\n\t"
+"v_fma_f64 v[120:121], v[120:121], v[122:123], 1.0\n\t"
+"v_fmac_f64_e32 %[a2], v[118:119], v[120:121]\n\t"
+"s_cmp_eq_u32 %[rem], 2\n\t"
+"s_cbranch_scc1 9f\n\t"
+"s_load_dwordx8 s[84:91], %[sp], s100\n\t"
+"s_add_u32 s100, s100, %[st]\n\t"
+"ds_read_b64 v[102:103], %[ca] offset:16\n\t"
+"s_waitcnt lgkmcnt(0)\n\t"
+"v_add_f64 v[106:107], %[q0], v[102:103]\n\t"
+"v_fmac_f64_e32 v[106:107], s[84:85], %[x00]\n\t"
+"v_fmac_f64_e32 v[106:107], s[86:87], %[x01]\n\t"
+"v_fmac_f64_e32 v[106:107], s[88:89], %[x02]\n\t"
+"v_fma_f64 v[106:107], s[90:91], %[x03], v[106:107] clamp\n\t"
+"v_fma_f64 v[108:109], %[nk], v[106:107], v[124:125]\n\t"
+"v_add_f64 v[110:111], v[108:109], %[nm]\n\t"
+"v_lshlrev_b16 v109, 3, v108\n\t"
+"v_fma_f64 v[110:111], v[106:107], %[nk], -v[110:111]\n\t"
+"ds_read_b64 v[106:107], v109\n\t"
+"v_add_f64 v[112:113], %[q1], v[102:103]\n\t"
+"v_fmac_f64_e32 v[112:113], s[84:85], %[x10]\n\t"
+"v_fmac_f64_e32 v[112:113], s[86:87], %[x11]\n\t"
+"v_fmac_f64_e32 v[112:113], s[88:89], %[x12]\n\t"
+"v_fma_f64 v[112:113], s[90:91], %[x13], v[112:113] clamp\n\t"
+"v_fma_f64 v[114:115], %[nk], v[112:113], v[124:125]\n\t"
+"v_add_f64 v[116:117], v[114:115], %[nm]\n\t"
+"v_lshlrev_b16 v115, 3, v114\n\t"
+"v_fma_f64 v[116:117], v[112:113], %[nk], -v[116:117]\n\t"
+"ds_read_b64 v[112:113], v115\n\t"
+"s_waitcnt lgkmcnt(1)\n\t"
+"v_lshl_add_u32 v107, v108, 8, v107\n\t"
+"v_fma_f64 v[108:109], %[c2], v[110:111], v[126:127]\n\t"
+"v_fma_f64 v[108:109], v[108:109], v[110:111], 1.0\n\t"
+"v_fmac_f64_e32 %[a0], v[106:107], v[108:109]\n\t"
+"v_add_f64 v[118:119], %[q2], v[102:103]\n\t"
+"v_fmac_f64_e32 v[118:119], s[84:85], %[x20]\n\t"
+"v_fmac_f64_e32 v[118:119], s[86:87], %[x21]\n\t"
+"v_fmac_f64_e32 v[118:119], s[88:89], %[x22]\n\t"
+"v_fma_f64 v[118:119], s[90:91], %[x23], v[118:119] clamp\n\t"
+"v_fma_f64 v[120:121], %[nk], v[118:119], v[124:125]\n\t"
+"v_add_f64 v[122:123], v[120:121], %[nm]\n\t"
+"v_lshlrev_b16 v121, 3, v120\n\t"
+"v_fma_f64 v[122:123], v[118:119], %[nk], -v[122:123]\n\t"
+"ds_read_b64 v[118:119], v121\n\t"
+"s_waitcnt lgkmcnt(1)\n\t"
+"v_lshl_add_u32 v113, v114, 8, v113\n\t"
+"v_fma_f64 v[114:115], %[c2], v[116:117], v[126:127]\n\t"
+"v_fma_f64 v[114:115], v[114:115], v[116:117], 1.0\n\t"
+"v_fmac_f64_e32 %[a1], v[112:113], v[114:115]\n\t"
+"s_waitcnt lgkmcnt(0)\n\t"
+"v_lshl_add_u32 v119, v120, 8, v119\n\t"
+"v_fma_f64 v[120:121], %[c2], v[122:123], v[126:127]\n\t"
+"v_fma_f64 v[120:121], v[120:121], v[122:123], 1.0\n\t"
+"v_fmac_f64_e32 %[a2], v[118:119], v[120:121]\n\t"
+"s_cmp_eq_u32 %[rem], 3\n\t"
+"s_cbranch_scc1 9f\n\t"
+"s_load_dwordx8 s[84:91], %[sp], s100\n\t"
+"s_add_u32 s100, s100, %[st]\n\t"
+"ds_read_b64 v[102:103], %[ca] offset:24\n\t"
+"s_waitcnt lgkmcnt(0)\n\t"
+"v_add_f64 v[106:107], %[q0], v[102:103]\n\t"
+"v_fmac_f64_e32 v[106:107], s[84:85], %[x00]\n\t"
+"v_fmac_f64_e32 v[106:107], s[86:87], %[x01]\n\t"
+"v_fmac_f64_e32 v[106:107], s[88:89], %[x02]\n\t"
+"v_fma_f64 v[106:107], s[90:91], %[x03], v[106:107] clamp\n\t"
+"v_fma_f64 v[108:109], %[nk], v[106:107], v[124:125]\n\t"
+"v_add_f64 v[110:111], v[108:109], %[nm]\n\t"
+"v_lshlrev_b16 v109, 3, v108\n\t"
+"v_fma_f64 v[110:111], v[106:107], %[nk], -v[110:111]\n\t"
+"ds_read_b64 v[106:107], v109\n\t"
+"v_add_f64 v[112:113], %[q1], v[102:103]\n\t"
+"v_fmac_f64_e32 v[112:113], s[84:85], %[x10]\n\t"
+"v_fmac_f64_e32 v[112:113], s[86:87], %[x11]\n\t"
+"v_fmac_f64_e32 v[112:113], s[88:89], %[x12]\n\t"
+"v_fma_f64 v[112:113], s[90:91], %[x13], v[112:113] clamp\n\t"
+"v_fma_f64 v[114:115], %[nk], v[112:113], v[124:125]\n\t"
+"v_add_f64 v[116:117], v[114:115], %[nm]\n\t"
+"v_lshlrev_b16 v115, 3, v114\n\t"
+"v_fma_f64 v[116:117], v[112:113], %[nk], -v[116:117]\n\t"
+"ds_read_b64 v[112:113], v115\n\t"
+"s_waitcnt lgkmcnt(1)\n\t"
+"v_lshl_add_u32 v107, v108, 8, v107\n\t"
+"v_fma_f64 v[108:109], %[c2], v[110:111], v[126:127]\n\t"
+"v_fma_f64 v[108:109], v[108:109], v[110:111], 1.0\n\t"
+"v_fmac_f64_e32 %[a0], v[106:107], v[108:109]\n\t"
+"v_add_f64 v[118:119], %[q2], v[102:103]\n\t"
+"v_fmac_f64_e32 v[118:119], s[84:85], %[x20]\n\t"
+"v_fmac_f64_e32 v[118:119], s[86:87], %[x21]\n\t"
+"v_fmac_f64_e32 v[118:119], s[88:89], %[x22]\n\t"
+"v_fma_f64 v[118:119], s[90:91], %[x23], v[118:119] clamp\n\t"
+"v_fma_f64 v[120:121], %[nk], v[118:119], v[124:125]\n\t"
+"v_add_f64 v[122:123], v[120:121], %[nm]\n\t"
+"v_lshlrev_b16 v121, 3, v120\n\t"
+"v_fma_f64 v[122:123], v[118:119], %[nk], -v[122:123]\n\t"
+"ds_read_b64 v[118:119], v121\n\t"
+"s_waitcnt lgkmcnt(1)\n\t"
+"v_lshl_add_u32 v113, v114, 8, v113\n\t"
+"v_fma_f64 v[114:115], %[c2], v[116:117], v[126:127]\n\t"
+"v_fma_f64 v[114:115], v[114:115], v[116:117], 1.0\n\t"
+"v_fmac_f64_e32 %[a1], v[112:113], v[114:115]\n\t"
+"s_waitcnt lgkmcnt(0)\n\t"
+"v_lshl_add_u32 v119, v120, 8, v119\n\t"
+"v_fma_f64 v[120:121], %[c2], v[122:123], v[126:127]\n\t"
+"v_fma_f64 v[120:121], v[120:121], v[122:123], 1.0\n\t"
+"v_fmac_f64_e32 %[a2], v[118:119], v[120:121]\n\t"
+"9:\n\t"
```

After: 460.8 Mcells/s, median of 6. +2.0%, better.
